# VIS4ROB-lab/HyperSLAM

Hardware: AMD Instinct MI355X
Metric: residual blocks linearised per second (LM iteration = linearise + Schur + solve + update), 128-control-point window (higher is better)
Workload: dtype f64

## Files before the change

hyperslam_amd/csrc/capi.hip:

```cpp
#include "host_tables.hpp"
#include "host_launch.hpp"
#include "tracker.hpp"

template <class Drop>
static int drop_rows(int n, Drop&& drop, std::vector<double>* stamp, std::vector<double>* meas, int width, std::vector<int32_t>* a = nullptr, std::vector<int32_t>* b = nullptr) {
  int w = 0;
  for (int i = 0; i < n; ++i) {
    if (drop(i)) continue;
    if (w != i) {
      (*stamp)[w] = (*stamp)[i];
      for (int c = 0; c < width; ++c) (*meas)[size_t(width) * w + c] = (*meas)[size_t(width) * i + c];
      if (a) (*a)[w] = (*a)[i];
      if (b) (*b)[w] = (*b)[i];
    }
    ++w;
  }
  stamp->resize(w), meas->resize(size_t(width) * w);
  if (a) a->resize(w);
  if (b) b->resize(w);
  return n - w;
}

extern "C" {

int hs_version(void) { return 1; }
const char* hs_arch(void) { return "gfx950"; }

int hs_create(int device, void* stream, hs_problem** out) {
  if (!out) return HS_ERR_INVALID;
  *out = nullptr;
  int count = 0;
  if (hipGetDeviceCount(&count) != hipSuccess || device < 0 || device >= count) return HS_ERR_DEVICE;
  hs_problem* p = new hs_problem();
  p->device = device;
  if (const char* e = std::getenv("HS_REFERENCE_LITERAL")) p->inertial_mode = std::atoi(e) ? HS_INERTIAL_AS_REFERENCE : HS_INERTIAL_EXACT;
  if (const char* e = std::getenv("HS_STAGE_TIMING")) p->stage_timing = std::atoi(e) != 0;
  if (const char* e = std::getenv("HS_HOST_TIMING")) p->host_timing = std::atoi(e) != 0;
  if (hipSetDevice(device) != hipSuccess) {
    delete p;
    return HS_ERR_DEVICE;
  }
  {
    int cus = 0;
    if (hipDeviceGetAttribute(&cus, hipDeviceAttributeMultiprocessorCount, device) == hipSuccess && cus > 0) p->n_cu = cus;
  }
  if (stream) {
    p->stream = static_cast<hipStream_t>(stream);
  } else {
    if (hipStreamCreateWithFlags(&p->stream, hipStreamNonBlocking) != hipSuccess) {
      delete p;
      return HS_ERR_DEVICE;
    }
    p->own_stream = true;
  }
  if (hipHostMalloc(reinterpret_cast<void**>(&p->h_state), sizeof(DevState), hipHostMallocDefault) != hipSuccess) {
    delete p;
    return HS_ERR_DEVICE;
  }
  warm_kernels(device);
  if (set_func_attributes(p) != HS_OK || ensure_side_stream(p) != HS_OK) {
    const std::string e = p->err;
    std::fprintf(stderr, "hyperslam_hip: %s\n", e.c_str());
    delete p;
    return HS_ERR_DEVICE;
  }
  *out = p;
  return HS_OK;
}

int hs_destroy(hs_problem* p) {
  if (!p) return HS_OK;
  if (p->host_timing && p->host_calls) {
    std::fprintf(stderr, "hs host timing over %d hs_solve calls [ms per call]: structure + tables %.4f, uploads %.4f, launches %.4f, wait %.4f\n", p->host_calls,
                 p->host_ms[0] / p->host_calls, p->host_ms[1] / p->host_calls, p->host_ms[2] / p->host_calls, p->host_ms[3] / p->host_calls);
    const size_t n = p->host_log.size() / 4, h = n / 2;
    double m[4] = {0, 0, 0, 0};
    for (size_t i = h; i < n; ++i)
      for (int c = 0; c < 4; ++c) m[c] += p->host_log[4 * i + c] / double(n - h);
    std::fprintf(stderr, "hs host timing, second half of the calls: structure + tables %.4f, uploads %.4f, launches %.4f, wait %.4f\n", m[0], m[1], m[2], m[3]);
    if (const char* e = std::getenv("HS_HOST_TIMING"); e && std::atoi(e) >= 2)
      for (size_t i = 0; i < n; ++i)
        std::fprintf(stderr, "hs host timing call %zu: structure + tables %.4f, uploads %.4f, launches %.4f, wait %.4f\n", i, p->host_log[4 * i],
                     p->host_log[4 * i + 1], p->host_log[4 * i + 2], p->host_log[4 * i + 3]);
  }
  if (p->scratch) hs_destroy(p->scratch), p->scratch = nullptr;
  (void)hipSetDevice(p->device);
  (void)hipStreamSynchronize(p->stream);
  for (hipEvent_t e : p->events) (void)hipEventDestroy(e);
  if (p->ev_fork) (void)hipEventDestroy(p->ev_fork);
  if (p->ev_join) (void)hipEventDestroy(p->ev_join);
  if (p->ev_irec) (void)hipEventDestroy(p->ev_irec);
  if (p->side) (void)hipStreamDestroy(p->side);
  if (p->h_state) (void)hipHostFree(p->h_state);
  if (p->h_result) (void)hipHostFree(p->h_result);
  if (p->rccl_comm && rccl_api()) (void)rccl_api()->CommDestroy(static_cast<ncclComm_t>(p->rccl_comm));
  if (p->own_stream) (void)hipStreamDestroy(p->stream);
  delete p;
  return HS_OK;
}

const char* hs_last_error(const hs_problem* p) { return p ? p->err.c_str() : "null handle"; }

static double knot_tolerance(double t0, double dt, int n_cp) {
  return std::max(1e-6 * dt, 8.0 * 2.220446049250313e-16 * std::max(std::fabs(t0), std::fabs(t0 + n_cp * dt)));
}

int hs_set_spline(hs_problem* p, int order, double t0, double dt, int n_cp, const double* cp, const uint8_t* cp_constant, int rc, int tc) {
  if (!p) return HS_ERR_INVALID;
  if (order < 2 || order > hsd::kMaxOrder) HS_FAIL(HS_ERR_INVALID, "spline order out of range");
  if (n_cp < order || !(dt > 0) || !cp) HS_FAIL(HS_ERR_INVALID, "need n_cp >= order, dt > 0 and a control-point table");
  const double knot_tol = knot_tolerance(t0, dt, n_cp);
  for (int j = 0; j < n_cp; ++j)
    if (!(std::fabs(cp[8 * j + 7] - (t0 + j * dt)) <= knot_tol))
      HS_FAIL(HS_ERR_KNOTS, "control-point stamps are not t0 + j dt (row " + std::to_string(j) + "): the spline basis is uniform, a table with a hole or non-uniform knots is refused");
  const bool same_structure = p->k == order && p->t0 == t0 && p->dt == dt && p->n_cp == n_cp && p->rot_const == (rc != 0) && p->trans_const == (tc != 0) &&
                              p->cp.size() == size_t(8) * n_cp;
  bool same_values = same_structure && std::memcmp(p->cp.data(), cp, sizeof(double) * 8 * n_cp) == 0;
  for (int j = 0; same_values && j < n_cp; ++j) same_values = p->cp_const[j] == (cp_constant ? cp_constant[j] : 0);
  if (same_values && !p->device_ahead) return HS_OK;
  p->k = order, p->t0 = t0, p->dt = dt, p->n_cp = n_cp;
  p->cp.assign(cp, cp + size_t(8) * n_cp);
  p->cp_const.assign(n_cp, 0);
  if (cp_constant) p->cp_const.assign(cp_constant, cp_constant + n_cp);
  p->rot_const = rc != 0, p->trans_const = tc != 0;
  p->touch(same_structure ? unsigned(hs_problem::vCp) : unsigned(hs_problem::kAll));
  return HS_OK;
}

static const char* kCameraShardMessage = "free camera blocks (hs_set_camera_constancy) are not supported on sharded handles (world > 1)";

int hs_set_cameras(hs_problem* p, int n, const double* T_bs, const double* intr, const double* dist) {
  if (!p) return HS_ERR_INVALID;
  if (n < 0 || n > 0xffff || (n && (!T_bs || !intr || !dist))) HS_FAIL(HS_ERR_INVALID, "bad camera table");
  const bool same_count = p->n_cam == n && p->cam.size() == size_t(kCamStride) * n;
  const std::vector<double> before = p->cam;
  p->n_cam = n;
  p->cam.assign(size_t(kCamStride) * n, 0.0);
  for (int i = 0; i < n; ++i) {
    double* c = &p->cam[size_t(kCamStride) * i];
    std::memcpy(c, T_bs + 7 * i, 56), std::memcpy(c + 7, intr + 4 * i, 32), std::memcpy(c + 11, dist + 4 * i, 32);
  }
  if (same_count && before == p->cam) return HS_OK;
  if (!same_count) p->cam_const.clear();
  p->touch(same_count ? unsigned(hs_problem::vCam) : unsigned(hs_problem::vCam | hs_problem::kVis));
  return HS_OK;
}

int hs_set_camera_constancy(hs_problem* p, int n, const uint8_t* constant) {
  if (!p) return HS_ERR_INVALID;
  std::vector<uint8_t> flags;
  if (constant) {
    if (n != p->n_cam) HS_FAIL(HS_ERR_INVALID, "hs_set_camera_constancy: n must equal the camera count of hs_set_cameras");
    flags.resize(size_t(3) * n);
    bool any_free = false;
    for (size_t i = 0; i < flags.size(); ++i) flags[i] = constant[i] ? 1 : 0, any_free |= !flags[i];
    if (!any_free) flags.clear();
  }
  if (flags == p->cam_const) return HS_OK;
  p->cam_const.swap(flags);
  p->touch(hs_problem::kTail);
  return HS_OK;
}

int hs_set_camera_estimation(hs_problem* p, int enabled) {
  if (!p) return HS_ERR_INVALID;
  const bool on = enabled != 0;
  if (on == p->cam_estimation) return HS_OK;
  p->cam_estimation = on;
  if (camera_columns(p, nullptr)) p->touch(hs_problem::kTail);
  return HS_OK;
}

int hs_get_cameras(hs_problem* p, double* T_bs, double* intr, double* dist) {
  if (!p) return HS_ERR_INVALID;
  for (int i = 0; i < p->n_cam; ++i) {
    const double* c = &p->cam[size_t(kCamStride) * i];
// ... 615 lines not shown
  }
  for (int d = 0; d < n_lm; ++d)
    if (lm_status[d])
      HS_FAIL(HS_ERR_NUMERIC, "hs_compute_covariance: rank deficient at landmark " + std::to_string(p->vs.table_of_dev[d]) +
                                  " (its observations do not fix all three coordinates)");
  p->cov_np = np, p->cov_ncb = ncb, p->cov_nb = nb, p->cov_nlm = n_lm;
  p->cov_valid = true;
  return HS_OK;
}

int hs_get_covariance(hs_problem* p, double* cp_blocks, double* cp_band, double* landmarks, double* border) {
  if (!p) return HS_ERR_INVALID;
  if (!p->cov_valid) HS_FAIL(HS_ERR_STATE, "hs_get_covariance: no covariance of the current state (call hs_compute_covariance after the last change)");
  const int np = p->cov_np, ncb = p->cov_ncb, nb = p->cov_nb, n_lm = p->cov_nlm, n_cp = np / 6, bw = ncb / 6;
  hipStream_t s = p->stream;
  std::vector<double> band, lm;
  if (cp_blocks || cp_band) {
    band.resize(size_t(np) * ncb);
    HIP_TRY(hipMemcpyAsync(band.data(), p->d_cov_band.p, band.size() * 8, hipMemcpyDeviceToHost, s));
  }
  if (landmarks && n_lm) {
    lm.resize(size_t(9) * n_lm);
    HIP_TRY(hipMemcpyAsync(lm.data(), p->d_cov_lm.p, lm.size() * 8, hipMemcpyDeviceToHost, s));
  }
  if (border && nb) HIP_TRY(hipMemcpyAsync(border, p->d_cov_bb.p, size_t(nb) * nb * 8, hipMemcpyDeviceToHost, s));
  HIP_TRY(hipStreamSynchronize(s));
  for (int i = 0; i < n_cp && (cp_blocks || cp_band); ++i)
    for (int j = 0; j < bw; ++j)
      for (int a = 0; a < 6; ++a)
        for (int b = 0; b < 6; ++b) {
          const double v = i + j < n_cp ? band[size_t(6 * i + a) * ncb + 6 * j + b] : 0.0;
          if (cp_band) cp_band[((size_t(i) * bw + j) * 6 + a) * 6 + b] = v;
          if (cp_blocks && j == 0) cp_blocks[(size_t(i) * 6 + a) * 6 + b] = v;
        }
  if (landmarks)
    for (int d = 0; d < n_lm; ++d) std::memcpy(landmarks + size_t(9) * p->vs.table_of_dev[d], lm.data() + size_t(9) * d, 9 * sizeof(double));
  return HS_OK;
}

int hs_sample_covariance(hs_problem* p, int n, const double* stamps, double* cov) {
  if (!p || n < 0 || (n && (!stamps || !cov))) return HS_ERR_INVALID;
  if (!p->cov_valid) HS_FAIL(HS_ERR_STATE, "hs_sample_covariance: no covariance of the current state (call hs_compute_covariance after the last change)");
  if (n == 0) return HS_OK;
  const int k = p->k, n_seg = p->n_cp - k + 1;
  for (int i = 0; i < n; ++i) {
    const int f = h_segment_first(stamps[i], p->t0, p->dt, k);
    if (f < 0 || f >= n_seg) HS_FAIL(HS_ERR_INVALID, "stamp outside the valid range of the spline");
  }
  hipStream_t s = p->stream;
  DBuf<double> d_st, d_out;
  std::vector<double> st(stamps, stamps + n);
  HIP_TRY(d_st.upload(st, s));
  HIP_TRY(d_out.reserve(size_t(36) * n));
  const int grid = (n + kBlock / 64 - 1) / (kBlock / 64);
  HS_ORDER_SWITCH(k, k_cov_sample<K><<<grid, kBlock, 0, s>>>(p->T, p->d_cov_band.p, n, d_st.p, d_out.p));
  HIP_TRY(hipGetLastError());
  HIP_TRY(hipMemcpyAsync(cov, d_out.p, size_t(36) * n * 8, hipMemcpyDeviceToHost, s));
  HIP_TRY(hipStreamSynchronize(s));
  return HS_OK;
}

int hs_set_weights(hs_problem* p, int type, const double* weights) {
  if (!p) return HS_ERR_INVALID;
  if (type < HS_PIXEL || type > HS_INERTIAL) HS_FAIL(HS_ERR_INVALID, "unknown factor type");
  const int nr = type == HS_PIXEL ? 2 : (type == HS_BEARING ? 1 : 6);
  if (weights)
    p->weights[type].assign(weights, weights + nr * nr);
  else
    p->weights[type].clear();
  return HS_OK;
}

int hs_set_guard(int enabled) {
  GuardRegistry::flag() = enabled != 0 ? 1 : 0;
  return HS_OK;
}

int hs_set_stage_timing(hs_problem* p, int enabled) {
  if (!p) return HS_ERR_INVALID;
  p->stage_timing = enabled != 0;
  return HS_OK;
}

int hs_solve(hs_problem* p, int max_iterations, hs_summary* summary, hs_iteration* iterations) {
  if (!p || !summary) return HS_ERR_INVALID;
  if (p->has_weights()) HS_FAIL(HS_ERR_INVALID, kWeightsMessage);
  if (max_iterations < 0 || max_iterations > kMaxIterations) HS_FAIL(HS_ERR_INVALID, "max_iterations out of range");
  if (camera_columns(p, nullptr)) {
    if (p->world > 1) HS_FAIL(HS_ERR_STATE, kCameraShardMessage);
    if (!p->cam_estimation)
      HS_FAIL(HS_ERR_STATE, "hs_solve: free camera blocks (hs_set_camera_constancy) are not supported by the solver in this version; "
                            "hs_reduced_system builds their system (DESIGN.md section 13)");
  }
  p->results_cached = false;
  p->cov_valid = false;
  int rc = prepare(p);
  if (rc) return rc;
  const bool spec = speculative_solve(p);
  const bool deferred = (fused_visual_only(p) || (spec && !commit_inline(p))) && !(p->T.debug_flags & 67108864);
  const bool fold = fold_decision_into_build(p, deferred);
  rc = reset_state(p, max_iterations, 1e4, spec ? (deferred ? 2 : 1) : (deferred ? 4 : 0));
  if (rc) return rc;
  hipStream_t s = p->stream;
  const auto host_t3 = std::chrono::steady_clock::now();
  const bool stages = p->stage_timing;
  const size_t n_ev = size_t(6) * max_iterations + 1;
  const size_t ev_cand = size_t(4) * max_iterations + 1;
  while (p->events.size() < n_ev) {
    hipEvent_t e;
    HIP_TRY(hipEventCreate(&e));
    p->events.push_back(e);
  }
  std::vector<hipEvent_t>& ev = p->events;
  HIP_TRY(hipEventRecord(ev[0], s));
  for (int it = 0; it < max_iterations; ++it) {
    if (it == 0 || !spec) {
      HS_ORDER_SWITCH(p->k, rc = launch_linearize<K>(p, true));
      if (rc) return rc;
    }
    if (stages && !p->fused) HIP_TRY(hipEventRecord(ev[4 * it + 1], s));
    hipEvent_t after_build = stages && p->fused ? ev[4 * it + 1] : nullptr;
    HS_ORDER_SWITCH(p->k, rc = launch_build<K>(p, after_build, it > 0, it > 0 && fold));
    if (rc) return rc;
    if (stages) HIP_TRY(hipEventRecord(ev[4 * it + 2], s));
    rc = launch_factor(p);
    if (rc) return rc;
    if (stages) HIP_TRY(hipEventRecord(ev[4 * it + 3], s));
    const bool lin_cand = spec && it + 1 < max_iterations;
    hipEvent_t* lin_ev = stages && lin_cand ? &ev[ev_cand + 2 * it] : nullptr;
    HS_ORDER_SWITCH(p->k, rc = launch_update<K>(p, lin_cand, deferred, lin_ev, fold && it + 1 < max_iterations));
    if (rc) return rc;
    if (deferred && it + 1 == max_iterations) launch_commit(p);
    if (stages || it + 1 == max_iterations) HIP_TRY(hipEventRecord(ev[4 * it + 4], s));
  }
  if (max_iterations == 0) {
    HS_ORDER_SWITCH(p->k, rc = launch_linearize<K>(p, false, true));
    if (rc) return rc;
    k_pack_exchange<<<1, kBlock, 0, s>>>(p->T, 0);
    rc = exchange(p, p->T.xbuf + p->T.xo_cost, 1);
    if (rc) return rc;
    k_cost_reduce<<<1, kBlock, 0, s>>>(p->T);
  }
  DevState& st = *p->h_state;
  const auto host_t4 = std::chrono::steady_clock::now();
  if (p->want_results) {
    const size_t n_cp8 = p->cp.size(), n_lm3 = p->lm.size(), n_b = p->has_imu ? p->bias_g.size() : 0, total = n_cp8 + n_lm3 + 2 * n_b + 3;
    if (total > p->h_result_cap) {
      if (p->h_result) (void)hipHostFree(p->h_result);
      p->h_result = nullptr, p->h_result_cap = 0;
      HIP_TRY(hipHostMalloc(reinterpret_cast<void**>(&p->h_result), 2 * total * sizeof(double), hipHostMallocDefault));
      p->h_result_cap = 2 * total;
    }
    double* h = p->h_result;
    HIP_TRY(hipMemcpyAsync(h, p->d_cp.p, n_cp8 * 8, hipMemcpyDeviceToHost, s));
    if (n_lm3) HIP_TRY(hipMemcpyAsync(h + n_cp8, p->d_lm.p, n_lm3 * 8, hipMemcpyDeviceToHost, s));
    if (n_b) {
      HIP_TRY(hipMemcpyAsync(h + n_cp8 + n_lm3, p->d_bias_g.p, n_b * 8, hipMemcpyDeviceToHost, s));
      HIP_TRY(hipMemcpyAsync(h + n_cp8 + n_lm3 + n_b, p->d_bias_a.p, n_b * 8, hipMemcpyDeviceToHost, s));
    }
    if (p->has_imu) HIP_TRY(hipMemcpyAsync(h + n_cp8 + n_lm3 + 2 * n_b, p->d_gravity.p, 24, hipMemcpyDeviceToHost, s));
  }
  if (p->T.nc && max_iterations > 0) HIP_TRY(hipMemcpyAsync(p->cam.data(), p->d_cam.p, p->cam.size() * 8, hipMemcpyDeviceToHost, s));
  HIP_TRY(hipMemcpyAsync(&st, p->d_state.p, sizeof(st), hipMemcpyDeviceToHost, s));
  HIP_TRY(hipStreamSynchronize(s));
  if (max_iterations > 0) p->device_ahead = true;
  p->results_cached = p->want_results;
  if (p->host_timing) {
    const auto host_t5 = std::chrono::steady_clock::now();
    const double tl = std::chrono::duration<double, std::milli>(host_t4 - host_t3).count(), tw = std::chrono::duration<double, std::milli>(host_t5 - host_t4).count();
    p->host_ms[2] += tl, p->host_ms[3] += tw;
    p->host_log.insert(p->host_log.end(), {p->host_prepare[0], p->host_prepare[1], tl, tw});
    p->host_prepare[0] = p->host_prepare[1] = 0;
    ++p->host_calls;
  }
  std::memset(summary, 0, sizeof(*summary));
  summary->initial_cost = st.records[0].cost;
  summary->final_cost = st.cost;
  summary->num_iterations = st.num_iterations;
  summary->num_successful_steps = st.num_successful;
  summary->termination = st.termination;
  summary->num_residual_blocks = p->T.n_vis + p->T.n_pri + p->T.n_ine;
  if (!stages) summary->linearize_ms = summary->schur_ms = summary->solve_ms = summary->update_ms = -1.0;
  for (int it = 0; stages && it < max_iterations; ++it) {
    float t[4] = {0, 0, 0, 0};
    for (int k = 0; k < 4; ++k) (void)hipEventElapsedTime(&t[k], ev[4 * it + k], ev[4 * it + k + 1]);
    summary->linearize_ms += t[0], summary->schur_ms += t[1], summary->solve_ms += t[2], summary->update_ms += t[3];
    if (spec && it + 1 < max_iterations) {
      float tc = 0;
      (void)hipEventElapsedTime(&tc, ev[ev_cand + 2 * it], ev[ev_cand + 2 * it + 1]);
      summary->linearize_ms += tc, summary->update_ms -= tc;
    }
  }
  if (max_iterations > 0) {
    float t = 0;
    (void)hipEventElapsedTime(&t, ev[0], ev[4 * max_iterations]);
    summary->total_ms = t;
  }
  if (iterations) {
    std::memset(iterations, 0, sizeof(hs_iteration) * (size_t(max_iterations) + 1));
    const int n = std::min(st.num_iterations, max_iterations);
    for (int i = 0; i <= n; ++i) iterations[i] = st.records[i];
  }
  if (st.chol_failed && st.termination == HS_FAILURE)
    p->err = st.chol_failed == 2 ? "two-ended solve: the partner workgroup did not arrive within 2 s" : "reduced system not positive definite";
  return guard_check(p);
}

#if HS_PROFILE_HOOKS
extern "C" int hs_debug_read(hs_problem* p, double* dst, int n) {
  if (!p || !dst) return HS_ERR_INVALID;
  HIP_TRY(hipMemcpyAsync(dst, p->d_xpart.p, size_t(n) * 8, hipMemcpyDeviceToHost, p->stream));
  HIP_TRY(hipStreamSynchronize(p->stream));
  return HS_OK;
}
#endif

int hs_snapshot(hs_problem* p) {
  if (!p) return HS_ERR_INVALID;
  int rc = prepare(p);
  if (rc) return rc;
  HIP_TRY(p->d_cp_snap.reserve(p->cp.size()));
  HIP_TRY(p->d_lm_snap.reserve(p->lm.size() + 1));
  HIP_TRY(hipMemcpyAsync(p->d_cp_snap.p, p->d_cp.p, p->cp.size() * 8, hipMemcpyDeviceToDevice, p->stream));
  if (p->n_lm) HIP_TRY(hipMemcpyAsync(p->d_lm_snap.p, p->d_lm.p, p->lm.size() * 8, hipMemcpyDeviceToDevice, p->stream));
  if (p->has_imu) {
    HIP_TRY(p->d_bias_g_snap.reserve(p->bias_g.size() + 1));
    HIP_TRY(p->d_bias_a_snap.reserve(p->bias_a.size() + 1));
    HIP_TRY(p->d_gravity_snap.reserve(3));
    HIP_TRY(hipMemcpyAsync(p->d_bias_g_snap.p, p->d_bias_g.p, p->bias_g.size() * 8, hipMemcpyDeviceToDevice, p->stream));
    HIP_TRY(hipMemcpyAsync(p->d_bias_a_snap.p, p->d_bias_a.p, p->bias_a.size() * 8, hipMemcpyDeviceToDevice, p->stream));
    HIP_TRY(hipMemcpyAsync(p->d_gravity_snap.p, p->d_gravity.p, 24, hipMemcpyDeviceToDevice, p->stream));
  }
  p->cam_snap = p->cam;
  p->has_snapshot = true;
  return HS_OK;
}

int hs_restore(hs_problem* p) {
  if (!p) return HS_ERR_INVALID;
  if (!p->has_snapshot || p->dirty) HS_FAIL(HS_ERR_STATE, "hs_restore without a valid hs_snapshot");
  p->results_cached = false;
  p->cov_valid = false;
  HIP_TRY(hipMemcpyAsync(p->d_cp.p, p->d_cp_snap.p, p->cp.size() * 8, hipMemcpyDeviceToDevice, p->stream));
  if (p->n_lm) HIP_TRY(hipMemcpyAsync(p->d_lm.p, p->d_lm_snap.p, p->lm.size() * 8, hipMemcpyDeviceToDevice, p->stream));
  if (p->has_imu) {
    HIP_TRY(hipMemcpyAsync(p->d_bias_g.p, p->d_bias_g_snap.p, p->bias_g.size() * 8, hipMemcpyDeviceToDevice, p->stream));
    HIP_TRY(hipMemcpyAsync(p->d_bias_a.p, p->d_bias_a_snap.p, p->bias_a.size() * 8, hipMemcpyDeviceToDevice, p->stream));
    HIP_TRY(hipMemcpyAsync(p->d_gravity.p, p->d_gravity_snap.p, 24, hipMemcpyDeviceToDevice, p->stream));
  }
  if (p->cam != p->cam_snap && p->cam.size() == p->cam_snap.size()) {
    p->cam = p->cam_snap;
    HIP_TRY(hipMemcpyAsync(p->d_cam.p, p->cam.data(), p->cam.size() * 8, hipMemcpyHostToDevice, p->stream));
    HIP_TRY(hipStreamSynchronize(p->stream));
  }
  return HS_OK;
}

int hs_rccl_unique_id(char id[128]) {
  static_assert(sizeof(ncclUniqueId) == 128, "ncclUniqueId is 128 bytes");
  if (!id) return HS_ERR_INVALID;
  RcclApi* api = rccl_api();
  if (!api) return HS_ERR_DEVICE;
  ncclUniqueId u;
  if (api->GetUniqueId(&u) != ncclSuccess) return HS_ERR_DEVICE;
  std::memcpy(id, &u, 128);
  return HS_OK;
}

int hs_rccl_init(hs_problem* p, const char id[128], int rank, int world) {
  if (!p || !id || world < 1 || rank < 0 || rank >= world) return HS_ERR_INVALID;
  RcclApi* api = rccl_api();
  if (!api) HS_FAIL(HS_ERR_DEVICE, "librccl.so could not be loaded");
  HIP_TRY(hipSetDevice(p->device));
  if (p->rccl_comm) {
    (void)api->CommDestroy(static_cast<ncclComm_t>(p->rccl_comm));
    p->rccl_comm = nullptr;
  }
  ncclUniqueId u;
  std::memcpy(&u, id, 128);
  ncclComm_t comm = nullptr;
  const ncclResult_t r = api->CommInitRank(&comm, world, u, rank);
  if (r != ncclSuccess) HS_FAIL(HS_ERR_DEVICE, std::string("ncclCommInitRank failed: ") + (api->GetErrorString ? api->GetErrorString(r) : "?"));
  p->rccl_comm = comm;
  return HS_OK;
}

int hs_rccl_shutdown(hs_problem* p) {
  if (!p) return HS_ERR_INVALID;
  if (p->rccl_comm && rccl_api()) {
    (void)hipStreamSynchronize(p->stream);
    (void)rccl_api()->CommDestroy(static_cast<ncclComm_t>(p->rccl_comm));
  }
  p->rccl_comm = nullptr;
  return HS_OK;
}

int hs_exchange_info(hs_problem* p, int32_t* rccl_ranks, int64_t* doubles_per_linearisation, int64_t* doubles_per_decision) {
  if (!p) return HS_ERR_INVALID;
  if (rccl_ranks) {
    int n = 0;
    if (p->rccl_comm && rccl_api() && rccl_api()->CommCount) {
      const ncclResult_t r = rccl_api()->CommCount(static_cast<ncclComm_t>(p->rccl_comm), &n);
      if (r != ncclSuccess) HS_FAIL(HS_ERR_DEVICE, "ncclCommCount failed");
    }
    *rccl_ranks = n;
  }
  if (doubles_per_linearisation) *doubles_per_linearisation = p->dirty ? 0 : p->T.x_count1;
  if (doubles_per_decision) *doubles_per_decision = 5;
  return HS_OK;
}

int hs_set_allreduce(hs_problem* p, hs_allreduce_fn fn, void* user) {
  if (!p) return HS_ERR_INVALID;
  p->allreduce = fn, p->allreduce_user = user;
  return HS_OK;
}

int hs_set_shard(hs_problem* p, int rank, int world, int min_band_blocks) {
  if (!p) return HS_ERR_INVALID;
  if (world < 1 || rank < 0 || rank >= world || min_band_blocks < 0) HS_FAIL(HS_ERR_INVALID, "bad shard description");
  p->rank = rank, p->world = world, p->min_bw = min_band_blocks;
  p->touch(hs_problem::kAll);
  return HS_OK;
}

int hs_band_blocks(hs_problem* p) {
  if (!p) return -1;
  if (prepare(p) != HS_OK) return -1;
  return p->T.bw;
}

// ... 601 lines not shown
```

hyperslam_amd/csrc/host_launch.hpp:

```cpp
#pragma once
#include "host_tables.hpp"

namespace {

int reset_state(hs_problem* p, int max_iterations, double radius, int spec = 0) {
  k_reset_state<<<1, 64, 0, p->stream>>>(p->d_state.p, max_iterations, radius, spec);
  HIP_TRY(hipGetLastError());
  return HS_OK;
}

size_t cp_lds_bytes(const hs_problem* p) { return size_t(8) * p->n_cp * sizeof(double); }
template <int K>
size_t lin_lds_bytes(const hs_problem* p) {
  return (cp_lds_bytes(p) <= 24 * 1024 ? cp_lds_bytes(p) : 0) + size_t(lin_block<K>()) * (8 + 12 * K + 2) * sizeof(double);
}

__global__ void k_noop() {}

static int ensure_side_stream(hs_problem* p) {
  if (!p->side) {
    HIP_TRY(hipStreamCreateWithFlags(&p->side, hipStreamNonBlocking));
    HIP_TRY(hipEventCreateWithFlags(&p->ev_fork, hipEventDisableTiming));
    HIP_TRY(hipEventCreateWithFlags(&p->ev_join, hipEventDisableTiming));
    HIP_TRY(hipEventCreateWithFlags(&p->ev_irec, hipEventDisableTiming));
// ... 15 lines not shown
    const int rc = ensure_side_stream(p);
    if (rc) return rc;
    HIP_TRY(hipEventRecord(p->ev_fork, s));
    HIP_TRY(hipStreamWaitEvent(p->side, p->ev_fork, 0));
  }
  if (T.n_vis && !p->fused) k_linearize_visual<K><<<p->nb_vis, lin_block<K>(), lin_lds_bytes<K>(p), s>>>(T, T.v_rec, T.v_pos, 1, T.cost_part, nullptr);
  if (T.n_vis && p->fused && visual_cost_only) k_cost_visual<K><<<p->nb_vis, kBlock, cp_lds_bytes(p), s>>>(T, T.cp, T.lm, T.cost_part);
  if (T.n_pri) k_linearize_prior<K><<<p->nb_pri, kBlock, cp_lds_bytes(p), s>>>(T, T.p_rec, T.cost_part + p->nb_vis, nullptr);
  if (T.n_ine)
    k_linearize_inertial<K, 4><<<p->nb_ine, kInertialBlock * K, cp_lds_bytes(p), p->side_imu ? p->side : s>>>(T, T.i_rec, 1, T.cost_part + p->nb_vis + p->nb_pri,
                                                                                                        nullptr);
  if (p->side_imu) HIP_TRY(hipEventRecord(p->ev_irec, p->side));
  HIP_TRY(hipGetLastError());
  return HS_OK;
}

struct RcclApi {
  void* lib = nullptr;
  ncclResult_t (*GetUniqueId)(ncclUniqueId*) = nullptr;
  ncclResult_t (*CommInitRank)(ncclComm_t*, int, ncclUniqueId, int) = nullptr;
  ncclResult_t (*AllReduce)(const void*, void*, size_t, ncclDataType_t, ncclRedOp_t, ncclComm_t, hipStream_t) = nullptr;
  ncclResult_t (*CommDestroy)(ncclComm_t) = nullptr;
  ncclResult_t (*CommCount)(const ncclComm_t, int*) = nullptr;
  const char* (*GetErrorString)(ncclResult_t) = nullptr;
};
static RcclApi* rccl_api() {
  static RcclApi api;
  static bool tried = false;
  if (!tried) {
    tried = true;
    for (const char* name : {"librccl.so.1", "librccl.so", "/opt/rocm/lib/librccl.so.1"}) {
      api.lib = dlopen(name, RTLD_NOW | RTLD_GLOBAL);
      if (api.lib) break;
    }
    if (api.lib) {
      api.GetUniqueId = reinterpret_cast<decltype(api.GetUniqueId)>(dlsym(api.lib, "ncclGetUniqueId"));
      api.CommInitRank = reinterpret_cast<decltype(api.CommInitRank)>(dlsym(api.lib, "ncclCommInitRank"));
      api.AllReduce = reinterpret_cast<decltype(api.AllReduce)>(dlsym(api.lib, "ncclAllReduce"));
      api.CommDestroy = reinterpret_cast<decltype(api.CommDestroy)>(dlsym(api.lib, "ncclCommDestroy"));
      api.GetErrorString = reinterpret_cast<decltype(api.GetErrorString)>(dlsym(api.lib, "ncclGetErrorString"));
      api.CommCount = reinterpret_cast<decltype(api.CommCount)>(dlsym(api.lib, "ncclCommCount"));
      if (!api.GetUniqueId || !api.CommInitRank || !api.AllReduce || !api.CommDestroy) api.lib = nullptr;
    }
  }
  return api.lib ? &api : nullptr;
}

int exchange(hs_problem* p, double* buf, int64_t count) {
  if (p->rccl_comm) {
    const ncclResult_t r = rccl_api()->AllReduce(buf, buf, size_t(count), ncclDouble, ncclSum, static_cast<ncclComm_t>(p->rccl_comm), p->stream);
    if (r != ncclSuccess) HS_FAIL(HS_ERR_DEVICE, std::string("ncclAllReduce failed: ") + (rccl_api()->GetErrorString ? rccl_api()->GetErrorString(r) : "?"));
    return HS_OK;
  }
  if (!p->allreduce) return HS_OK;
  if (p->allreduce(p->allreduce_user, buf, count, p->stream) != 0) HS_FAIL(HS_ERR_DEVICE, "all-reduce hook reported a failure");
  return HS_OK;
}

static int border_zero_wgs(const Tables& T) { return std::min(64, (T.nb * T.nb + T.nb + kPbThreads - 1) / kPbThreads); }

static bool factor_two_ended_la(const hs_problem* p) {
  const Tables& T = p->T;
  const int n_blk = T.np / 6;
  return T.nb == 0 && !(T.debug_flags & 4) && la_compute_waves(T.bw) > 0 && !HS_AB(T.debug_flags, 131072) && n_blk >= 4 * T.bw && T.Sb2 && !(T.debug_flags & 2048);
}

int mfma_window_tiles(int bw);
static bool factor_two_ended_any(const hs_problem* p) {
  const Tables& T = p->T;
  const int n_blk = T.np / 6;
  const bool la_ok = !(T.debug_flags & 4) && la_compute_waves(T.bw) > 0;
  const int nt = HS_AB(T.debug_flags, 131072) ? mfma_window_tiles(T.bw) : 0;
  if (T.nc) return false;
  return (la_ok || nt) && (T.nb == 0 || (!nt && !(T.debug_flags & 536870912) && (T.nb + kBorderCols - 1) / kBorderCols <= 512)) && n_blk >= 4 * T.bw && T.Sb2 &&
         !(T.debug_flags & 2048);
}
static bool use_dense_mx(const hs_problem* p, int* f0) {
  const Tables& T = p->T;
  const int n_blk = T.np / 6;
  *f0 = (T.debug_flags & 262144) ? 0 : std::min(p->frozen_prefix, n_blk - 1);
  return !factor_two_ended_any(p) && !HS_AB(T.debug_flags, 131072) && dense_mx_fits(n_blk - *f0, T.nb) && !(T.debug_flags & 8);
}

template <int K>
int launch_build(hs_problem* p, hipEvent_t after_build = nullptr, bool scaling_fixed = false, bool fold = false) {
  const Tables& T = p->T;
  hipStream_t s = p->stream;
  p->bookkeep = false;
  const bool fused = p->fused;
  const bool pair = !fused && T.n_lm > 0 && p->n_group_wg > 0 && p->n_group_wg + p->n_seg_wg <= 2048 && !(T.debug_flags & 1024);
  const bool side_imu = p->side_imu;
  const bool fork = !fused && T.n_lm > 0 && !pair && !side_imu;
  if (fused && fold) {
    Tables Tf = T;
    Tf.fold_decision = 1, Tf.fold_epoch = ++p->join_epoch;
    k_build_visual<K><<<p->nb_vis + 1, kBlock, p->build_lds, s>>>(Tf, p->build_R, p->build_L, 1);
  } else if (fused)
    k_build_visual<K><<<p->nb_vis, kBlock, p->build_lds, s>>>(T, p->build_R, p->build_L, 1);
  if (fused && T.wide_q) k_landmark_gram_wide<<<landmark_gram_wide_grid(T.sp.n_cp, T.bw), kGramWideThreads, 0, s>>>(T);
  if (fused && after_build) HIP_TRY(hipEventRecord(after_build, s));
  if (fork) {
    const int rc = ensure_side_stream(p);
    if (rc) return rc;
    HIP_TRY(hipEventRecord(p->ev_fork, s));
    HIP_TRY(hipStreamWaitEvent(p->side, p->ev_fork, 0));
  }
  hipStream_t sb = side_imu ? p->side : s;
  const bool gather_flag = side_imu && T.nb && !p->allreduce && !p->rccl_comm && p->world == 1 && !(T.debug_flags & 16384) &&
                           !(T.debug_flags & 8388608);
  const unsigned gather_epoch = gather_flag ? ++p->join_epoch : 0u;
  if (side_imu && T.nb) {
    k_border_pb<K><<<dim3(T.sp.n_cp + border_zero_wgs(T), p->n_split), kPbThreads, 0, sb>>>(T);
    Tables Tg = T;
    Tg.gather_epoch = gather_epoch;
    k_border_bb<K><<<T.n_bias, kBlock, 0, sb>>>(Tg);
    HIP_TRY(hipEventRecord(p->ev_join, p->side));
  }
  bool irec_ready = !side_imu;
  auto need_irec = [&]() -> hipError_t {
    if (irec_ready) return hipSuccess;
    irec_ready = true;
    return hipStreamWaitEvent(s, p->ev_irec, 0);
  };
  if (!pair && !(side_imu && T.n_lm) && p->n_seg_wg) {
    HIP_TRY(need_irec());
    k_seg_gram<K><<<p->n_seg_wg, kBlock, kSegStage * sizeof(double), fork ? p->side : s>>>(T);
  }
  if (fork) HIP_TRY(hipEventRecord(p->ev_join, p->side));
  if (T.n_lm && !fused) {
    const int grid = (T.n_lm + kBlock / 64 - 1) / (kBlock / 64);
    if (6 * T.bw <= 128)
      k_landmark<K, 2, 2><<<grid, kBlock, 0, s>>>(T);
    else if (T.debug_flags & 4194304)
      k_landmark<K, 4, 1><<<grid, kBlock, 0, s>>>(T);
    else
      k_landmark_rows<K, 4><<<T.n_lm, kBlock, 0, s>>>(T);
  }
  if (T.n_lm && p->n_group_wg && !fused) {
    const int ntile = T.bw * (T.bw + 1) / 2;
    const int batch = std::max(2, std::min(kGroupBatch, int(48 * 1024 / (size_t(18) * T.bw * sizeof(double)))));
    const size_t lds = std::max((size_t(batch) * 18 * T.bw + 4 * batch) * sizeof(double), size_t(128) * 42 * sizeof(double));
    const dim3 grid(p->n_group_wg);
    if (pair) {
      HIP_TRY(need_irec());
      const size_t lds2 = std::max(lds, kSegStage * sizeof(double));
      const dim3 grid2(p->n_group_wg + p->n_seg_wg);
      if (ntile <= kBlock)
        k_gram_pair<K, 1><<<grid2, kBlock, lds2, s>>>(T, batch, p->n_group_wg);
      else if (ntile <= 2 * kBlock)
        k_gram_pair<K, 2><<<grid2, kBlock, lds2, s>>>(T, batch, p->n_group_wg);
      else
        k_gram_pair<K, 4><<<grid2, kBlock, lds2, s>>>(T, batch, p->n_group_wg);
    } else if (ntile <= kBlock)
      k_group_gram<1><<<grid, kBlock, lds, s>>>(T, batch);
    else if (ntile <= 2 * kBlock)
      k_group_gram<2><<<grid, kBlock, lds, s>>>(T, batch);
    else
      k_group_gram<4><<<grid, kBlock, lds, s>>>(T, batch);
  }
  if (side_imu && T.n_lm && !pair && p->n_seg_wg) {
    HIP_TRY(need_irec());
    k_seg_gram<K><<<p->n_seg_wg, kBlock, kSegStage * sizeof(double), s>>>(T);
  }
  if (fork) HIP_TRY(hipStreamWaitEvent(s, p->ev_join, 0));
  Tables Ta = T;
  const bool dense_mx = use_dense_mx(p, &Ta.dense_f0);
  const bool direct = scaling_fixed && fused && !T.nb && !p->allreduce && !p->rccl_comm && p->world == 1 && (factor_two_ended_la(p) || dense_mx) &&
                      !(T.debug_flags & 4096);
  if (direct && dense_mx) Ta.dense = p->d_dense_ut.p + size_t(kDenseLd) * kDenseLd;
  if (fused && T.bw * (T.bw + 1) / 2 > kBlock)
    k_assemble_wide<K><<<dim3(T.sp.n_cp, 6), kAsmWideThreads, 0, s>>>(Ta, direct ? 1 : 0);
  else
    k_assemble<K><<<dim3(T.sp.n_cp, 6), kAsmThreads, 0, s>>>(Ta, direct ? 1 : 0);
  if (direct) {
    p->bookkeep = true;
    HIP_TRY(hipGetLastError());
    return HS_OK;
  }
// ... 280 lines not shown
static bool speculative_solve(const hs_problem* p) {
  const Tables& T = p->T;
  return !p->fused && T.n_vis > 0 && !T.n_pri && !T.n_ine && !T.nb && !(T.debug_flags & 1073741824);
}
static bool fused_visual_only(const hs_problem* p) {
  const Tables& T = p->T;
  return p->fused && !T.n_pri && !T.n_ine && !T.nb;
}

static bool fold_decision_into_build(const hs_problem* p, bool deferred_commit) {
  return fused_visual_only(p) && deferred_commit && !p->allreduce && !p->rccl_comm && p->world == 1 && !(p->T.debug_flags & 32768);
}

static bool commit_inline(const hs_problem* p) {
  const Tables& T = p->T;
  return !p->allreduce && !p->rccl_comm && 8 * T.sp.n_cp + 3 * T.n_lm + 8 * T.n_bias <= kCommitInline && !(T.debug_flags & 16777216);
}

template <int K>
int launch_update(hs_problem* p, bool linearize_candidate = false, bool deferred_commit = false, hipEvent_t* lin_events = nullptr, bool fold_next = false) {
  const Tables& T = p->T;
  hipStream_t s = p->stream;
  const bool local_decision = !p->allreduce && !p->rccl_comm;
  const bool inline_commit = commit_inline(p) && !deferred_commit;
  const bool cps_here = p->fused && deferred_commit;
  const int decide_here = inline_commit ? 2 : local_decision ? (cps_here ? 3 : 1) : 0;
  const bool merged = p->fused && local_decision && !(T.debug_flags & 134217728);
  Tables calib_tables[2];
  if (T.nc) {
    k_calib_candidate<<<1, kBlock, 0, s>>>(T, p->d_cam_cand.p, T.n_norm_part);
    calib_tables[0] = calib_tables[1] = T;
    calib_tables[0].cam = p->d_cam_cand.p, calib_tables[1].n_norm_part = T.n_norm_part + 1;
  }
  const Tables &Tc = T.nc ? calib_tables[0] : T, &Td = T.nc ? calib_tables[1] : T;
  if (p->fused) {
    const int nb_pri = merged && T.n_pri ? p->nb_pri : 0, nb_ine = merged && T.n_ine ? p->nb_ine : 0;
    const size_t lds = std::max(size_t(update_lds_doubles(T.bw, p->build_R, p->build_L)), size_t(8 * T.sp.n_cp + 8 * T.n_bias + 4)) * 8;
    if (T.nc)
      k_update_visual<K, true><<<p->nb_vis + T.n_norm_part + nb_pri + nb_ine, kBlock, lds, s>>>(Tc, p->build_R, p->build_L, p->nb_vis, nb_pri, nb_ine);
    else
      k_update_visual<K><<<p->nb_vis + T.n_norm_part + nb_pri + nb_ine, kBlock, lds, s>>>(T, p->build_R, p->build_L, p->nb_vis, nb_pri, nb_ine);
    if (T.n_pri && !merged) k_cost_prior<K><<<p->nb_pri, kBlock, cp_lds_bytes(p), s>>>(T, T.cp_cand, T.cand_part + p->nb_vis);
    if (T.n_ine && !merged)
      k_cost_inertial<K, 4><<<p->nb_ine, kInertialBlock, cp_lds_bytes(p), s>>>(T, T.cp_cand, T.bias_g_cand, T.bias_a_cand, T.gravity_cand,
                                                                          T.cand_part + p->nb_vis + p->nb_pri);
  } else if (T.nc)
    k_backsub_retract<true><<<T.n_lm_part + T.n_norm_part, kBlock, 0, s>>>(T);
  else
    k_backsub_retract<false><<<T.n_lm_part + T.n_norm_part, kBlock, 0, s>>>(T);
  if (p->fused) {
  } else if (linearize_candidate) {
    if (lin_events) HIP_TRY(hipEventRecord(lin_events[0], s));
    k_linearize_visual<K><<<p->nb_vis, lin_block<K>(), lin_lds_bytes<K>(p), s>>>(T, nullptr, T.v_pos, 1, T.cand_part, nullptr, T.cp_cand, T.lm_cand);
    if (lin_events) HIP_TRY(hipEventRecord(lin_events[1], s));
  } else if ((T.n_ine || T.n_pri) && !(T.debug_flags & 33554432)) {
    k_cost_all<K, 4><<<p->nb_vis + p->nb_pri + p->nb_ine, kBlock, cp_lds_bytes(p), s>>>(Tc, T.cp_cand, T.lm_cand, T.bias_g_cand, T.bias_a_cand, T.gravity_cand,
                                                                                       T.cand_part, p->nb_vis, p->nb_pri);
  } else {
    if (T.n_vis) k_cost_visual<K><<<p->nb_vis, kBlock, cp_lds_bytes(p), s>>>(Tc, T.cp_cand, T.lm_cand, T.cand_part);
    if (T.n_pri) k_cost_prior<K><<<p->nb_pri, kBlock, cp_lds_bytes(p), s>>>(T, T.cp_cand, T.cand_part + p->nb_vis);
    if (T.n_ine)
      k_cost_inertial<K, 4><<<p->nb_ine, kInertialBlock, cp_lds_bytes(p), s>>>(T, T.cp_cand, T.bias_g_cand, T.bias_a_cand, T.gravity_cand,
                                                                          T.cand_part + p->nb_vis + p->nb_pri);
  }
  if (fold_next) return HS_OK;
  k_pack_decision<<<1, kBlock, 0, s>>>(Td, decide_here);
  HIP_TRY(hipGetLastError());
  const int rc = exchange(p, T.xbuf + T.xo_dec, 5);
  if (rc) return rc;
  if (!local_decision) k_decide<<<1, kBlock, 0, s>>>(T, cps_here ? 1 : 0);
  const int nb_commit = std::max((std::max(8 * T.sp.n_cp, 3 * T.n_lm) + kBlock - 1) / kBlock, 1);
  if (!inline_commit && !deferred_commit) k_commit<<<nb_commit, kBlock, 0, s>>>(T);
  if (T.nc) k_calib_commit<<<1, kBlock, 0, s>>>(T, p->d_cam.p, p->d_cam_cand.p);
  HIP_TRY(hipGetLastError());
  return HS_OK;
}

static void launch_commit(hs_problem* p) {
  const Tables& T = p->T;
  const int nb_commit = std::max((std::max(8 * T.sp.n_cp, 3 * T.n_lm) + kBlock - 1) / kBlock, 1);
  k_commit<<<nb_commit, kBlock, 0, p->stream>>>(T);
}

template <int K>
static void warm_kernels_of_order() {
  hipFuncAttributes fa;
  const void* kernels[] = {
      reinterpret_cast<const void*>(&k_build_visual<K>), reinterpret_cast<const void*>(&k_update_visual<K>), reinterpret_cast<const void*>(&k_linearize_visual<K>), reinterpret_cast<const void*>(&k_linearize_prior<K>),
      reinterpret_cast<const void*>(&k_linearize_inertial<K, 4>), reinterpret_cast<const void*>(&k_landmark<K, 2, 2>),
      reinterpret_cast<const void*>(&k_landmark<K, 4, 1>), reinterpret_cast<const void*>(&k_landmark_rows<K, 4>),
      reinterpret_cast<const void*>(&k_gram_pair<K, 1>), reinterpret_cast<const void*>(&k_gram_pair<K, 2>), reinterpret_cast<const void*>(&k_gram_pair<K, 4>),
      reinterpret_cast<const void*>(&k_seg_gram<K>), reinterpret_cast<const void*>(&k_assemble<K>), reinterpret_cast<const void*>(&k_assemble_wide<K>), reinterpret_cast<const void*>(&k_border_pb<K>),
      reinterpret_cast<const void*>(&k_border_bb<K>), reinterpret_cast<const void*>(&k_cost_visual<K>), reinterpret_cast<const void*>(&k_cost_prior<K>),
      reinterpret_cast<const void*>(&k_cost_inertial<K, 4>), reinterpret_cast<const void*>(&k_cost_all<K, 4>),
      reinterpret_cast<const void*>(&k_process_tracks<K>), reinterpret_cast<const void*>(&k_sample_trajectory<K>)};
  for (const void* k : kernels) (void)hipFuncGetAttributes(&fa, k);
}
static void warm_kernels(int device) {
  static std::mutex mu;
  static std::vector<int> done;
  std::lock_guard<std::mutex> lock(mu);
  if (std::find(done.begin(), done.end(), device) != done.end()) return;
  done.push_back(device);
  hipFuncAttributes fa;
  const void* kernels[] = {
      reinterpret_cast<const void*>(&k_group_gram<1>), reinterpret_cast<const void*>(&k_group_gram<2>), reinterpret_cast<const void*>(&k_group_gram<4>),
      reinterpret_cast<const void*>(&k_pack_exchange), reinterpret_cast<const void*>(&k_cost_reduce), reinterpret_cast<const void*>(&k_finalize_reduced),
      reinterpret_cast<const void*>(&k_finalize_border), reinterpret_cast<const void*>(&k_reduce_partials), reinterpret_cast<const void*>(&k_factor_decoupled_rows),
      reinterpret_cast<const void*>(&k_dense_factor), reinterpret_cast<const void*>(&k_dense_solve_mx), reinterpret_cast<const void*>(&k_band_factor_wide), reinterpret_cast<const void*>(&k_band_factor<1>),
      reinterpret_cast<const void*>(&k_band_factor<2>), reinterpret_cast<const void*>(&k_band_factor_la<1, 3>), reinterpret_cast<const void*>(&k_band_factor_la<1, 4>),
      reinterpret_cast<const void*>(&k_band_backward), reinterpret_cast<const void*>(&k_band_backward_sb), reinterpret_cast<const void*>(&k_border_forward),
      reinterpret_cast<const void*>(&k_border_forward2),
      reinterpret_cast<const void*>(&k_border_schur), reinterpret_cast<const void*>(&k_border_solve), reinterpret_cast<const void*>(&k_border_solve_reg<3>), reinterpret_cast<const void*>(&k_border_solve_reg<4>),
      reinterpret_cast<const void*>(&k_border_solve_reg<5>), reinterpret_cast<const void*>(&k_border_solve_reg<6>), reinterpret_cast<const void*>(&k_border_solve_reg<7>),
      reinterpret_cast<const void*>(&k_border_solve_reg<8>), reinterpret_cast<const void*>(&k_border_apply), reinterpret_cast<const void*>(&k_backsub_retract<false>),
      reinterpret_cast<const void*>(&k_pack_decision), reinterpret_cast<const void*>(&k_decide), reinterpret_cast<const void*>(&k_commit),
      reinterpret_cast<const void*>(&k_reset_state), reinterpret_cast<const void*>(&k_scatter_uploads)};
  for (const void* k : kernels) (void)hipFuncGetAttributes(&fa, k);
  warm_kernels_of_order<4>();
  warm_kernels_of_order<5>();
  warm_kernels_of_order<6>();
}

int set_func_attributes(hs_problem* p) {
  hipFuncAttributes fa;
  HIP_TRY(hipFuncGetAttributes(&fa, reinterpret_cast<const void*>(&k_band_factor<2>)));
  p->chol_lds_max = 160 * 1024 - int(fa.sharedSizeBytes);
  HIP_TRY(hipFuncSetAttribute(reinterpret_cast<const void*>(&k_band_factor<1>), hipFuncAttributeMaxDynamicSharedMemorySize, p->chol_lds_max));
  HIP_TRY(hipFuncSetAttribute(reinterpret_cast<const void*>(&k_band_factor<2>), hipFuncAttributeMaxDynamicSharedMemorySize, p->chol_lds_max));
  HIP_TRY(hipFuncSetAttribute(reinterpret_cast<const void*>(&k_band_factor_la<1, 3>), hipFuncAttributeMaxDynamicSharedMemorySize, p->chol_lds_max));
  HIP_TRY(hipFuncSetAttribute(reinterpret_cast<const void*>(&k_band_factor_la<1, 4>), hipFuncAttributeMaxDynamicSharedMemorySize, p->chol_lds_max));
  for (int k = 4; k <= 6; ++k) HS_ORDER_SWITCH(k, {
    HIP_TRY(hipFuncSetAttribute(reinterpret_cast<const void*>(&k_seg_gram<K>), hipFuncAttributeMaxDynamicSharedMemorySize, 64 * 1024));
    HIP_TRY(hipFuncSetAttribute(reinterpret_cast<const void*>(&k_gram_pair<K, 1>), hipFuncAttributeMaxDynamicSharedMemorySize, 64 * 1024));
    HIP_TRY(hipFuncSetAttribute(reinterpret_cast<const void*>(&k_gram_pair<K, 2>), hipFuncAttributeMaxDynamicSharedMemorySize, 64 * 1024));
    HIP_TRY(hipFuncSetAttribute(reinterpret_cast<const void*>(&k_gram_pair<K, 4>), hipFuncAttributeMaxDynamicSharedMemorySize, 64 * 1024));
    HIP_TRY(hipFuncSetAttribute(reinterpret_cast<const void*>(&k_build_visual<K>), hipFuncAttributeMaxDynamicSharedMemorySize, 158 * 1024));
    HIP_TRY(hipFuncSetAttribute(reinterpret_cast<const void*>(&k_update_visual<K>), hipFuncAttributeMaxDynamicSharedMemorySize, 158 * 1024));
    HIP_TRY(hipFuncSetAttribute(reinterpret_cast<const void*>(&k_update_visual<K, true>), hipFuncAttributeMaxDynamicSharedMemorySize, 158 * 1024));
    HIP_TRY(hipFuncSetAttribute(reinterpret_cast<const void*>(&k_linearize_visual<K>), hipFuncAttributeMaxDynamicSharedMemorySize, 150 * 1024));
  });
  HIP_TRY(hipFuncSetAttribute(reinterpret_cast<const void*>(&k_dense_solve_mx), hipFuncAttributeMaxDynamicSharedMemorySize, int(kDxLdsDoubles * sizeof(double))));
  HIP_TRY(hipFuncSetAttribute(reinterpret_cast<const void*>(&k_border_solve_reg<5>), hipFuncAttributeMaxDynamicSharedMemorySize, 160 * 1024 - 1024));
  HIP_TRY(hipFuncSetAttribute(reinterpret_cast<const void*>(&k_border_solve_reg<6>), hipFuncAttributeMaxDynamicSharedMemorySize, 160 * 1024 - 1024));
  HIP_TRY(hipFuncSetAttribute(reinterpret_cast<const void*>(&k_border_solve_reg<7>), hipFuncAttributeMaxDynamicSharedMemorySize, 160 * 1024 - 1024));
  HIP_TRY(hipFuncSetAttribute(reinterpret_cast<const void*>(&k_border_solve_reg<8>), hipFuncAttributeMaxDynamicSharedMemorySize, 160 * 1024 - 1024));
  HIP_TRY(hipFuncSetAttribute(reinterpret_cast<const void*>(&k_border_forward), hipFuncAttributeMaxDynamicSharedMemorySize, 150 * 1024));
  HIP_TRY(hipFuncSetAttribute(reinterpret_cast<const void*>(&k_border_forward2), hipFuncAttributeMaxDynamicSharedMemorySize, 150 * 1024));
#if HS_PROFILE_HOOKS
  HIP_TRY(hipFuncSetAttribute(reinterpret_cast<const void*>(&k_band_backward2), hipFuncAttributeMaxDynamicSharedMemorySize, 150 * 1024));
#endif
  HIP_TRY(hipFuncSetAttribute(reinterpret_cast<const void*>(&k_band_backward_sb), hipFuncAttributeMaxDynamicSharedMemorySize, 150 * 1024));
  HIP_TRY(hipFuncSetAttribute(reinterpret_cast<const void*>(&k_band_backward), hipFuncAttributeMaxDynamicSharedMemorySize, 150 * 1024));
  HIP_TRY(hipFuncSetAttribute(reinterpret_cast<const void*>(&k_border_solve), hipFuncAttributeMaxDynamicSharedMemorySize, 150 * 1024));
  return HS_OK;
}

}
```

hyperslam_amd/csrc/host_structure.hpp:

```cpp
#pragma once
#include <algorithm>
#include <cmath>
#include <cstdint>
#include <numeric>
#include <string>
#include <vector>

#include "../../include/hyperslam_hip.h"
#include "device_math.hpp"

namespace hs {

inline double h_binom(int n, int r) {
  if (r < 0 || r > n) return 0.0;
  double v = 1.0;
  for (int i = 1; i <= r; ++i) v = v * (n - r + i) / i;
  return v;
}

inline hsd::BasisCoef make_basis_coef(int k) {
  hsd::BasisCoef b;
  for (double& v : b.c) v = 0.0;
  std::vector<double> M(size_t(k) * k, 0.0);
  double fact = 1.0;
// ... 107 lines not shown
    std::vector<int>& start = vs->scratch_start;
    start.assign(in.n_cp + 2, 0);
    for (int t = 0; t < in.n_lm; ++t) start[std::min(cf[t], in.n_cp) + 1]++;
    for (int c = 0; c <= in.n_cp; ++c) start[c + 1] += start[c];
    vs->table_of_dev.resize(in.n_lm), vs->dev_of_table.resize(in.n_lm);
    for (int t = 0; t < in.n_lm; ++t) {
      const int d = start[std::min(cf[t], in.n_cp)]++;
      vs->table_of_dev[d] = t, vs->dev_of_table[t] = d;
    }
  }
  vs->lm_cfirst.resize(in.n_lm), vs->lm_ncp.resize(in.n_lm), vs->lm_yoff.resize(in.n_lm + 1), vs->lm_ptr.resize(in.n_lm + 1);
  vs->lm_yoff[0] = 0, vs->lm_ptr[0] = 0;
  vs->bw = in.k;
  for (int d = 0; d < in.n_lm; ++d) {
    const int t = vs->table_of_dev[d];
    if (cl[t] >= 0) {
      vs->lm_cfirst[d] = cf[t];
      vs->lm_ncp[d] = cl[t] - cf[t] + 1;
      vs->bw = std::max(vs->bw, vs->lm_ncp[d]);
    } else {
      vs->lm_cfirst[d] = in.n_cp;
      vs->lm_ncp[d] = 0;
    }
    vs->lm_yoff[d + 1] = vs->lm_yoff[d] + 18 * vs->lm_ncp[d];
    vs->lm_ptr[d + 1] = vs->lm_ptr[d] + cnt[t];
    cnt[t] = vs->lm_ptr[d];
  }
  vs->y_total = vs->lm_yoff[in.n_lm];
  vs->cf_ptr.assign(in.n_cp + 2, 0);
  for (int c = 0, d = 0; c <= in.n_cp + 1; ++c) {
    while (d < in.n_lm && vs->lm_cfirst[d] < c) ++d;
    vs->cf_ptr[c] = d;
  }
  vs->table_type.resize(n), vs->table_idx.resize(n), vs->lm_dev.resize(n), vs->first.resize(n), vs->pos.resize(n);
  auto pass_b = [&](const int32_t* lm, int count, int offset, int type) {
    for (int j = 0; j < count; ++j) {
      const int t = lm[j], q = cnt[t]++;
      vs->table_type[q] = type, vs->table_idx[q] = j, vs->lm_dev[q] = vs->dev_of_table[t], vs->first[q] = first[offset + j];
    }
  };
  pass_b(in.px_lm, in.n_px, 0, HS_PIXEL), pass_b(in.br_lm, in.n_br, in.n_px, HS_BEARING);
  {
    std::vector<int>& cur = vs->scratch_start;
    cur.assign(vs->seg_ptr.begin(), vs->seg_ptr.end() - 1);
    for (int q = 0; q < n; ++q) vs->pos[q] = cur[vs->first[q]]++;
  }
  return true;
}

inline bool build_chunks(const VisualStructure& vs, int n_cp, int R, int L, std::vector<int>* ch_ptr, std::vector<int>* gw_ptr, std::vector<int>* gw_cf,
                         std::vector<int>* ch_desc = nullptr) {
  int n_obs = int(vs.lm_ptr.size()) - 1;
  while (n_obs > 0 && vs.lm_ptr[n_obs] == vs.lm_ptr[n_obs - 1]) --n_obs;
  ch_ptr->clear(), gw_cf->clear();
  gw_ptr->assign(n_cp + 1, 0);
  for (int c = 0; c < n_cp; ++c) {
    const int d0 = std::min(vs.cf_ptr[c], n_obs), d1 = std::min(vs.cf_ptr[c + 1], n_obs);
    (*gw_ptr)[c] = int(gw_cf->size());
    if (d1 <= d0) continue;
    int d = d0;
    while (d < d1) {
      if (vs.lm_ptr[d + 1] - vs.lm_ptr[d] > R) return false;
      ch_ptr->push_back(d), gw_cf->push_back(c);
      int cnt = 0, e = d;
      while (e < d1 && e - d < L && cnt + (vs.lm_ptr[e + 1] - vs.lm_ptr[e]) <= R) cnt += vs.lm_ptr[e + 1] - vs.lm_ptr[e], ++e;
      d = e;
    }
  }
  (*gw_ptr)[n_cp] = int(gw_cf->size());
  ch_ptr->push_back(n_obs);
  gw_cf->push_back(0);
  if (ch_desc) {
    const int n = int(ch_ptr->size()) - 1;
    ch_desc->assign(size_t(8) * std::max(n, 1), 0);
    for (int w = 0; w < n; ++w) {
      const int lo = (*ch_ptr)[w], hi = (*ch_ptr)[w + 1];
      int* d = ch_desc->data() + 8 * w;
      d[0] = lo, d[1] = hi - lo, d[2] = vs.lm_cfirst[lo], d[3] = vs.lm_ptr[lo], d[4] = vs.lm_ptr[hi] - vs.lm_ptr[lo], d[5] = w;
    }
  }
  return true;
}

inline void order_chunks_for_dispatch(const VisualStructure& vs, int k, int n_cu, std::vector<int>* ch_desc, int n) {
  if (n <= 1 || n_cu <= 0) return;
  std::vector<int> weight(n), order(n);
  std::vector<int> cnt;
  for (int c = 0; c < n; ++c) {
    const int* d = ch_desc->data() + 8 * c;
    cnt.assign(size_t(vs.bw) + k + 1, 0);
    for (int q = d[3]; q < d[3] + d[4]; ++q) {
      const int o = vs.first[q] - d[2];
      if (o >= 0 && o < vs.bw) cnt[o]++;
    }
    int run = 0, best = 0;
    for (int o = 0; o < vs.bw + k; ++o) {
      run += (o < vs.bw ? cnt[o] : 0) - (o >= k ? cnt[o - k] : 0);
      best = std::max(best, run);
    }
    weight[c] = best, order[c] = c;
  }
  std::stable_sort(order.begin(), order.end(), [&](int a, int b) { return weight[a] > weight[b]; });
  std::vector<int> slot_chunk(n, -1);
  if (n > n_cu && n <= 2 * n_cu) {
    const int n_lone = 2 * n_cu - n, n_pair = n - n_cu;
    for (int i = 0; i < n_lone; ++i) slot_chunk[n_pair + i] = order[i];
    for (int i = 0; i < n_pair; ++i) slot_chunk[i] = order[n_lone + i], slot_chunk[n_cu + i] = order[n - 1 - i];
  } else {
    for (int i = 0; i < n; ++i) slot_chunk[i] = order[i];
  }
  std::vector<int> out(ch_desc->size(), 0);
  for (int w = 0; w < n; ++w) std::copy(ch_desc->begin() + 8 * slot_chunk[w], ch_desc->begin() + 8 * slot_chunk[w] + 8, out.begin() + 8 * w);
  ch_desc->swap(out);
}

template <class LdsBytes>
inline bool choose_build_geometry(int k, int R0, int L0, size_t lds_two, size_t lds_one, LdsBytes lds_bytes, int* R, int* L) {
  for (const size_t cap : {lds_two, lds_one}) {
    int r = R0, l = L0;
    while (lds_bytes(r, l) > cap && l > 4) --l;
    while (lds_bytes(r, l) > cap && r > 64) r -= 32;
    if (lds_bytes(r, l) <= cap) {
      *R = r, *L = l;
      return true;
    }
  }
  (void)k;
  return false;
}

}
```

hyperslam_amd/csrc/host_tables.hpp:

```cpp
#pragma once
#include <dlfcn.h>
#include <hip/hip_runtime.h>
#include <rccl/rccl.h>

#include <cstdio>
#include <cstdlib>
#include <chrono>
#include <cstring>
#include <string>
#include <mutex>
#include <vector>

#include "host_structure.hpp"
#include "kernels.hpp"

using namespace hs;

namespace {

struct UploadBatch {
  struct Seg {
    unsigned long long dst, off, bytes;
  };
  std::vector<Seg> segs;
// ... 176 lines not shown
  void touch(unsigned what) { changed |= what, dirty = true, cov_valid = false; }
  bool device_ahead = false;

  int k = 0, n_cp = 0;
  double t0 = 0, dt = 0;
  std::vector<double> cp;
  std::vector<uint8_t> cp_const;
  int rot_const = 0, trans_const = 0;
  int n_cam = 0;
  std::vector<double> cam;
  std::vector<uint8_t> cam_const;
  bool cam_estimation = false;
  std::vector<double> cam_snap;
  int n_sensor = 0;
  std::vector<double> sensor;
  int n_lm = 0;
  std::vector<double> lm;
  std::vector<uint8_t> lm_const;
  std::vector<double> px_stamp, px_meas, br_stamp, br_meas, pr_stamp, pr_meas, in_stamp, in_meas;
  std::vector<int32_t> px_lm, px_cam, br_lm, br_cam, pr_sensor;
  bool has_imu = false;
  double imu_T_bs[7], imu_i_g[6], imu_i_a[6], imu_S_g[9], imu_X_a[9];
  int kb = 4, n_bias = 0;
  double bias_t0 = 0, bias_dt = 1;
  std::vector<double> bias_g, bias_a;
  int bias_const = 0;
  double gravity[3] = {0, 0, -9.80665};
  int gravity_const = 1;
  int inertial_mode = HS_INERTIAL_AS_REFERENCE;
  hs_problem* scratch = nullptr;
  int frozen_prefix = 0;
  bool stage_timing = false;
  std::vector<double> weights[4];
  bool has_weights() const { return !weights[0].empty() || !weights[1].empty() || !weights[2].empty() || !weights[3].empty(); }
  UploadBatch batch;
  bool host_timing = false;
  double host_ms[5] = {0, 0, 0, 0, 0};
  int host_calls = 0;
  std::vector<double> host_log;
  double host_prepare[2] = {0, 0};
  double* h_result = nullptr;
  size_t h_result_cap = 0;
  bool want_results = false, results_cached = false;
  size_t vb_len = 0;
  int zeroed_np = -1, zeroed_ncb = -1;
  const void* zeroed_ptr[5] = {nullptr, nullptr, nullptr, nullptr, nullptr};

  VisualStructure vs;
  std::vector<int> pr_order;
  std::vector<int> pr_first, pr_seg_ptr;

  DBuf<double> d_cp, d_cp_cand, d_cam, d_sensor, d_lm, d_lm_cand;
  DBuf<uint8_t> d_cp_const, d_lm_const;
  DBuf<int> d_lm_ptr, d_lm_cfirst, d_lm_ncp, d_lm_yoff, d_cf_ptr;
  DBuf<double> d_lm_scale, d_lm_L, d_lm_yhat, d_lm_sb, d_lm_D2, d_lm_part, d_lm_gmax, d_gabs, d_Y;
  DBuf<double> d_v_stamp, d_v_meas, d_v_rec, d_v_rec_alt;
  DBuf<int> d_v_lm, d_v_info, d_v_first, d_v_pos, d_v_seg_ptr, d_v_dbgpos;
  DBuf<double> d_p_stamp, d_p_meas, d_p_rec;
  DBuf<double> d_i_stamp, d_i_meas, d_i_rec, d_bias_g, d_bias_a, d_bias_g_cand, d_bias_a_cand, d_gravity, d_gravity_cand;
  DBuf<int> d_i_first, d_i_first_bias, d_i_seg_ptr;
  DBuf<ImuParams> d_imu;
  std::vector<int> in_order, in_first, in_first_bias, in_seg_ptr, in_bias_ptr;
  int nb_ine = 0;
  DBuf<int> d_p_sensor, d_p_first, d_p_seg_ptr;
  DBuf<double> d_scale_p, d_Sb, d_Ub, d_Ubk, d_g_s, d_g_full, d_D2p, d_step_p, d_delta_p;
  DBuf<double> d_cost_part, d_cand_part, d_norm_part, d_dbg, d_dbg_cost;
  DBuf<DevState> d_state;
  DBuf<double> d_xbuf, d_xpart, d_segP, d_grpQ, d_Qw, d_Yt, d_gravity_part;
  int yt_stride = 0;
  bool wide_q = false;
  DBuf<double> d_Vb, d_Vb2, d_yt, d_yt2;
  DBuf<double> d_Sb2, d_g2, d_Ub2, d_Ubk2, d_ybuf2, d_win, d_xsol;
  DBuf<unsigned> d_join;
  DBuf<double> d_dense_ut;
  DBuf<double> d_bf_handover;
  unsigned join_epoch = 0;
  DBuf<int> d_gw_ptr, d_gw_cf, d_sw_ptr, d_sw_seg;
  int n_seg_wg = 0, n_group_wg = 0;
  bool fused = false;
  int dense_border_nb = -1;
  bool bookkeep = false;
  int build_R = 0, build_L = 0;
  size_t build_lds = 0;
  DBuf<int> d_ch_ptr, d_ch_desc;
  DBuf<double> d_ch_gmax;
  std::vector<int> h_ch_ptr, h_gw_ptr, h_gw_cf, h_ch_desc;
  DBuf<double> d_ybuf, d_scale_b, d_Spb, d_Sbb, d_gb_s, d_D2b, d_Zb, d_Cb, d_hb, d_xb, d_delta_b, d_bias_g_snap, d_bias_a_snap, d_gravity_snap;
  DBuf<int> d_i_bias_ptr, d_bfwd_start;
  int n_split = 1;
  int rank = 0, world = 1, min_bw = 0;
  DBuf<double> d_cp_snap, d_lm_snap;
  bool has_snapshot = false;
  DevState* h_state = nullptr;
  bool cov_valid = false;
  int cov_np = 0, cov_ncb = 0, cov_nb = 0, cov_nlm = 0;
  DBuf<double> d_cov_U, d_cov_sig, d_cov_Z, d_cov_X, d_cov_C, d_cov_Li, d_cov_band, d_cov_pb, d_cov_bb, d_cov_lm;
  DBuf<uint8_t> d_cov_const;
  DBuf<int> d_cov_status, d_cov_lm_status;
  int nc = 0;
  std::vector<int> calib_map;
  DBuf<int> d_calib_map;
  DBuf<double> d_calib_rec, d_calib_Yc, d_calib_part, d_cam_cand;
  DBuf<int> d_calib_bfwd;
  std::vector<hipEvent_t> events;
  hipStream_t side = nullptr;
  hipEvent_t ev_fork = nullptr, ev_join = nullptr, ev_irec = nullptr;
  bool side_imu = false;
  Tables T;
  int nb_vis = 0, nb_pri = 0, nb_cp = 0;
  int chol_lds_max = 64 * 1024;
  hs_allreduce_fn allreduce = nullptr;
  void* allreduce_user = nullptr;
  void* rccl_comm = nullptr;
};

static const char* kWeightsMessage =
    "a weight matrix is set (hs_set_weights): weights are applied by hs_linearize / hs_cost_function_evaluate; the solver runs the "
    "reference's production configuration, weights = nullptr (optimizer.cpp:191,214,236,255)";

#define HS_AB(flags, bit) (HS_PROFILE_HOOKS && ((flags) & (bit)))

#define HS_ORDER_SWITCH(k, ...)    \
  do {                             \
    if ((k) == 4) {                \
      constexpr int K = 4;         \
      __VA_ARGS__;                 \
    } else if ((k) == 5) {         \
      constexpr int K = 5;         \
      __VA_ARGS__;                 \
    } else {                       \
      constexpr int K = 6;         \
      __VA_ARGS__;                 \
    }                              \
  } while (0)

#define HS_FAIL(code, msg) \
  do {                     \
    p->err = (msg);        \
    return (code);         \
  } while (0)
#define HIP_TRY(expr)                                                                             \
  do {                                                                                            \
    const hipError_t e__ = (expr);                                                                \
    if (e__ != hipSuccess) {                                                                      \
      p->err = std::string(#expr) + ": " + hipGetErrorString(e__);                                \
      return HS_ERR_DEVICE;                                                                       \
    }                                                                                             \
  } while (0)

namespace {

int mfma_window_tiles(int bw);

static int camera_columns(const hs_problem* p, std::vector<int>* map) {
  if (map) map->clear();
  if (p->cam_const.empty()) return 0;
  std::vector<uint8_t> used(p->n_cam, 0);
  for (int32_t c : p->px_cam)
    if (c >= 0 && c < p->n_cam) used[c] = 1;
  for (int32_t c : p->br_cam)
    if (c >= 0 && c < p->n_cam) used[c] = 1;
  static const int first[3] = {0, 6, 10}, size[3] = {6, 4, 4};
  int n = 0;
  for (int c = 0; c < p->n_cam; ++c)
    for (int b = 0; b < 3; ++b)
      if (used[c] && !p->cam_const[3 * c + b])
        for (int j = 0; j < size[b]; ++j, ++n)
          if (map) map->push_back(c << 8 | (first[b] + j));
  return n;
}

static int upload_values(hs_problem* p, unsigned what) {
  hipStream_t s = p->stream;
  if (what & hs_problem::vCp) {
    HIP_TRY(p->d_cp.upload(p->cp, s));
    HIP_TRY(p->d_cp_cand.reserve(p->cp.size()));
// ... 295 lines not shown
                                  " control points, at most " + std::to_string(150 * 1024 / (6 * 8 * 8)) + " (6 n_cp x 8 doubles within 150 KiB)");
    if (nbd + 1 > 128 && (size_t(nbd + 1) * (nbd + 1) + nbd) * sizeof(double) > size_t(150) * 1024)
      HS_FAIL(HS_ERR_INVALID, "too many border unknowns for the LDS-resident dense solve of the border system: " + std::to_string(nbi) +
                                  " bias / gravity + " + std::to_string(p->nc) + " free camera coordinates = " + std::to_string(nbd) +
                                  ", at most 137 (hs_set_camera_estimation)");
  }
  if (nbi && size_t(np) * 8 * 8 > 150 * 1024) HS_FAIL(HS_ERR_INVALID, "window too long for the LDS-resident border forward sweep");
  if (nbi + 1 > 128 && (size_t(nbi + 1) * (nbi + 1) + nbi) * sizeof(double) > size_t(150) * 1024)
    HS_FAIL(HS_ERR_INVALID, "too many border unknowns (bias control points) for the LDS-resident dense solve of the border system: at most 22 bias control points per window");
  const int x_count0 = np * (ncb + 3) + np * nbd + nbd * nbd + nbd + 1 + p->world;
  const int x_count1 = x_count0 + 2 * p->nc;
  if (p->nc) {
    HIP_TRY(p->d_calib_map.upload(p->calib_map, s));
    HIP_TRY(p->d_calib_rec.reserve(size_t(std::max(n_vis, 1)) * (40 + 12 * k)));
    HIP_TRY(p->d_calib_Yc.reserve(size_t(std::max(p->n_lm, 1)) * 3 * p->nc));
    const int n_parts = (n_vis + kCalibRowChunk - 1) / kCalibRowChunk + (p->n_lm + kCalibLmChunk - 1) / kCalibLmChunk;
    HIP_TRY(p->d_calib_part.reserve(size_t(std::max(n_parts, 1)) * (p->nc * p->nc + 2 * p->nc)));
    HIP_TRY(p->d_cam_cand.reserve(size_t(kCamStride) * std::max(p->n_cam, 1)));
    HIP_TRY(p->d_calib_bfwd.upload(std::vector<int>((nbd + kBorderCols - 1) / kBorderCols + kSchurTile, 0), s));
  }
  HIP_TRY(p->d_ybuf.reserve(np));
  HIP_TRY(p->d_scale_b.reserve(nbd + 1));
  HIP_TRY(p->d_Spb.reserve(size_t(np) * nbd + 1));
  HIP_TRY(p->d_Sbb.reserve(size_t(nbd) * nbd + 1));
  HIP_TRY(p->d_gb_s.reserve(nbd + 1));
  HIP_TRY(p->d_D2b.reserve(nbd + 1));
  HIP_TRY(p->d_Zb.reserve(size_t(np) * nbd + 1));
  HIP_TRY(p->d_Cb.reserve(size_t(nbd) * nbd + 1));
  HIP_TRY(p->d_hb.reserve(nbd + 1));
  HIP_TRY(p->d_xb.reserve(nbd + 1));
  HIP_TRY(p->d_delta_b.reserve(nbd + 1));
  HIP_TRY(p->d_xbuf.reserve(size_t(x_count1) + 8));
  HIP_TRY(p->d_gravity_part.reserve(size_t(5) * std::max(p->n_bias, 1)));
  {
    const size_t nv = size_t(np) * ncb, pad = 64, vb_len = std::max(nv, size_t(576) * ((size_t(p->n_cp) + 3) / 4 + 1));
    p->vb_len = vb_len;
    HIP_TRY(p->d_Sb2.reserve(nv));
    for (DBuf<double>* b : {&p->d_Vb, &p->d_Vb2}) HIP_TRY(b->reserve(vb_len + pad));
    for (DBuf<double>* b : {&p->d_yt, &p->d_yt2}) HIP_TRY(b->reserve(size_t(np) + pad));
    const void* now[5] = {p->d_Sb2.p, p->d_Vb.p, p->d_Vb2.p, p->d_yt.p, p->d_yt2.p};
    if (p->zeroed_np != np || p->zeroed_ncb != ncb || std::memcmp(now, p->zeroed_ptr, sizeof(now)) != 0) {
      HIP_TRY(hipMemsetAsync(p->d_Sb2.p, 0, p->d_Sb2.cap * sizeof(double), s));
      for (DBuf<double>* b : {&p->d_Vb, &p->d_Vb2}) HIP_TRY(hipMemsetAsync(b->p + vb_len, 0, pad * sizeof(double), s));
      for (DBuf<double>* b : {&p->d_yt, &p->d_yt2}) HIP_TRY(hipMemsetAsync(b->p + np, 0, pad * sizeof(double), s));
      p->zeroed_np = np, p->zeroed_ncb = ncb, std::memcpy(p->zeroed_ptr, now, sizeof(now));
    }
  }
  HIP_TRY(p->d_g2.reserve(np));
  HIP_TRY(p->d_Ub2.reserve(size_t(np) * ncb));
  HIP_TRY(p->d_Ubk2.reserve(size_t(p->n_cp) * 24));
  HIP_TRY(p->d_ybuf2.reserve(np));
  HIP_TRY(p->d_xsol.reserve(np));
  HIP_TRY(p->d_win.reserve(size_t(6) * vs.bw * (ncb + 1)));
  HIP_TRY(p->d_dense_ut.reserve(size_t(2) * kDenseLd * kDenseLd));
  if (!p->d_join.p) {
    HIP_TRY(p->d_join.reserve(kGatherFlag + kProgressStride));
    HIP_TRY(hipMemsetAsync(p->d_join.p, 0, (kGatherFlag + kProgressStride) * sizeof(unsigned), s));
    p->join_epoch = 0;
  }
  p->n_split = std::max(1, std::min(16, 2048 / std::max(p->n_cp, 1)));
  HIP_TRY(p->d_xpart.reserve(size_t(x_count1) * p->n_split));
  {
    const int n_seg_ = p->n_cp - k + 1, nca = 6 * k, ntile = vs.bw * (vs.bw + 1) / 2;
    std::vector<int> sw_ptr(n_seg_ + 1, 0), sw_seg;
    for (int f = 0; f < n_seg_; ++f) {
      const int load = (p->fused ? 0 : vs.seg_ptr[f + 1] - vs.seg_ptr[f]) + 3 * (p->pr_seg_ptr[f + 1] - p->pr_seg_ptr[f]) +
                       (p->in_seg_ptr.empty() ? 0 : 3 * (p->in_seg_ptr[f + 1] - p->in_seg_ptr[f]));
      const int nw = p->fused ? (load + 95) / 96 : std::max(1, (load + 95) / 96);
      sw_ptr[f + 1] = sw_ptr[f] + nw;
      for (int w = 0; w < nw; ++w) sw_seg.push_back(f);
    }
    p->n_seg_wg = sw_ptr[n_seg_];
    sw_seg.push_back(0);
    HIP_TRY(p->d_sw_ptr.upload(sw_ptr, s));
    HIP_TRY(p->d_sw_seg.upload(sw_seg, s));
    const int per_wg = 12;
    std::vector<int> gw_ptr(p->n_cp + 1, 0), gw_cf;
    if (!(what & hs_problem::kVis)) {
    } else if (p->fused) {
      HIP_TRY(p->d_gw_ptr.upload(p->h_gw_ptr, s));
      HIP_TRY(p->d_gw_cf.upload(p->h_gw_cf, s));
      HIP_TRY(p->d_ch_ptr.upload(p->h_ch_ptr, s));
      HIP_TRY(p->d_ch_desc.upload(p->h_ch_desc, s));
      p->n_group_wg = int(p->h_ch_ptr.size()) - 1;
    } else {
      for (int c = 0; c < p->n_cp; ++c) {
        const int cnt = vs.cf_ptr[c + 1] - vs.cf_ptr[c], nw = (cnt + per_wg - 1) / per_wg;
        gw_ptr[c + 1] = gw_ptr[c] + nw;
        for (int w = 0; w < nw; ++w) gw_cf.push_back(c);
      }
      p->n_group_wg = gw_ptr[p->n_cp];
      gw_cf.push_back(0);
      HIP_TRY(p->d_gw_ptr.upload(gw_ptr, s));
      HIP_TRY(p->d_gw_cf.upload(gw_cf, s));
    }
    HIP_TRY(p->d_segP.reserve(size_t(p->n_seg_wg) * (size_t(nca) * nca + nca) + 1));
    HIP_TRY(p->d_grpQ.reserve(size_t(p->n_group_wg) * (size_t(ntile) * 36 + (p->fused ? 3 : 1) * 6 * vs.bw) + 1));
    {
      const char* env = std::getenv("HS_WIDE_Q");
      p->wide_q = p->fused && ntile > kBlock && !(env && std::atoi(env) == 0);
      if (p->wide_q) {
        HIP_TRY(p->d_Qw.reserve(size_t(6) * p->n_cp * (6 * vs.bw + 1) + 1));
        p->yt_stride = (p->n_lm + 63) / 64 * 64;
        HIP_TRY(p->d_Yt.reserve(size_t(18) * p->n_cp * p->yt_stride + 2));
      }
    }
  }
  HIP_TRY(p->d_state.reserve(1));

  Tables& T = p->T;
  std::memset(&T, 0, sizeof(T));
  p->dense_border_nb = -1;
  T.sp = Spline{k, p->n_cp, p->t0, p->dt, 1.0 / p->dt, p->rot_const, p->trans_const};
  T.basis = make_basis_coef(k);
  T.cp = p->d_cp.p, T.cp_cand = p->d_cp_cand.p, T.cp_const = p->d_cp_const.p;
  T.cam = p->d_cam.p, T.n_cam = p->n_cam, T.sensor = p->d_sensor.p;
  T.n_lm = p->n_lm, T.lm = p->d_lm.p, T.lm_cand = p->d_lm_cand.p, T.lm_const = p->d_lm_const.p;
  T.lm_ptr = p->d_lm_ptr.p, T.lm_cfirst = p->d_lm_cfirst.p, T.lm_ncp = p->d_lm_ncp.p, T.lm_yoff = p->d_lm_yoff.p, T.cf_ptr = p->d_cf_ptr.p;
  T.lm_scale = p->d_lm_scale.p, T.lm_L = p->d_lm_L.p, T.lm_yhat = p->d_lm_yhat.p, T.lm_sb = p->d_lm_sb.p, T.lm_D2 = p->d_lm_D2.p;
  T.lm_part = p->d_lm_part.p, T.n_lm_part = p->fused ? p->nb_vis : (p->n_lm + kBlock / 64 - 1) / (kBlock / 64), T.lm_gmax = p->d_lm_gmax.p, T.Y = p->d_Y.p;
  {
    int n_obs = p->n_lm;
    while (n_obs > 0 && vs.lm_ptr[n_obs] == vs.lm_ptr[n_obs - 1]) --n_obs;
    T.n_obs_lm = n_obs;
  }
  T.n_vis = n_vis, T.v_stamp = p->d_v_stamp.p, T.v_meas = p->d_v_meas.p, T.v_lm = p->d_v_lm.p, T.v_info = p->d_v_info.p;
  T.v_first = p->d_v_first.p, T.v_pos = p->d_v_pos.p, T.v_rec = p->d_v_rec.p, T.v_rec_alt = p->d_v_rec_alt.p, T.v_seg_ptr = p->d_v_seg_ptr.p;
  T.n_pri = n_pri, T.p_stamp = p->d_p_stamp.p, T.p_meas = p->d_p_meas.p, T.p_sensor = p->d_p_sensor.p, T.p_first = p->d_p_first.p;
  T.p_rec = p->d_p_rec.p, T.p_seg_ptr = p->d_p_seg_ptr.p;
  T.n_ine = n_ine, T.i_stamp = p->d_i_stamp.p, T.i_meas = p->d_i_meas.p, T.i_first = p->d_i_first.p, T.i_first_bias = p->d_i_first_bias.p;
  T.i_rec = p->d_i_rec.p, T.i_seg_ptr = p->d_i_seg_ptr.p, T.imu = p->d_imu.p;
  T.bias_basis = make_basis_coef(p->kb), T.kb = p->kb, T.n_bias = p->has_imu ? p->n_bias : 0, T.bias_t0 = p->bias_t0, T.bias_dt = p->bias_dt;
  T.bias_g = p->d_bias_g.p, T.bias_a = p->d_bias_a.p, T.bias_g_cand = p->d_bias_g_cand.p, T.bias_a_cand = p->d_bias_a_cand.p;
  T.gravity = p->d_gravity.p, T.gravity_cand = p->d_gravity_cand.p, T.bias_const = p->bias_const, T.gravity_const = p->gravity_const;
  T.inertial_literal = p->inertial_mode == HS_INERTIAL_AS_REFERENCE;
  T.nb = (p->has_imu ? 6 * p->n_bias + 2 : 0) + p->nc;
  T.nc = p->nc, T.calib_map = p->d_calib_map.p, T.calib_rec = p->d_calib_rec.p, T.calib_Yc = p->d_calib_Yc.p, T.calib_part = p->d_calib_part.p;
  T.n_seg = n_seg, T.bw = vs.bw, T.np = np;
  T.scale_p = p->d_scale_p.p, T.Sb = p->d_Sb.p, T.Ub = p->d_Ub.p, T.Ubk = p->d_Ubk.p, T.g_s = p->d_g_s.p, T.g_full = p->d_g_full.p, T.D2p = p->d_D2p.p, T.gabs = p->d_gabs.p;
  T.step_p = p->d_step_p.p, T.delta_p = p->d_delta_p.p;
  T.cost_part = p->d_cost_part.p, T.cand_part = p->d_cand_part.p, T.n_cost_part = p->nb_vis + p->nb_pri + p->nb_ine;
  if (size_t(T.n_cost_part) > p->d_cost_part.cap || size_t(T.n_cost_part) > p->d_cand_part.cap)
    HS_FAIL(HS_ERR_DEVICE, "internal: cost partial tables shorter than the grids that write them");
  T.norm_part = p->d_norm_part.p, T.n_norm_part = nb_norm;
  T.xbuf = p->d_xbuf.p;
  T.xpart = p->d_xpart.p, T.gravity_part = p->d_gravity_part.p, T.segP = p->d_segP.p, T.grpQ = p->d_grpQ.p, T.Qw = p->d_Qw.p, T.wide_q = p->wide_q && n_vis > 0 ? 1 : 0, T.Yt = p->d_Yt.p, T.yt_stride = p->yt_stride, T.gw_ptr = p->d_gw_ptr.p, T.gw_cf = p->d_gw_cf.p, T.sw_ptr = p->d_sw_ptr.p, T.sw_seg = p->d_sw_seg.p;
  T.xo_g = np * ncb, T.xo_gs = T.xo_g + np, T.xo_dj = T.xo_gs + np, T.xo_pb = T.xo_dj + np, T.xo_bb = T.xo_pb + np * nbd;
  T.xo_gb = T.xo_bb + nbd * nbd, T.xo_cost = T.xo_gb + nbd, T.xo_gmax = T.xo_cost + 1;
  T.ybuf = p->d_ybuf.p, T.ybuf2 = nullptr, T.y_split = np;
  T.fj[0] = FactorJob{T.Sb, T.g_s, T.Ub, T.Ubk, T.ybuf, nullptr, np / 6, -1};
  T.fj[1] = FactorJob{nullptr, nullptr, nullptr, nullptr, nullptr, nullptr, 0, -1};
  T.xsol = p->d_xsol.p, T.join_flag = p->d_join.p, T.join_epoch = 0;
  T.debug_flags = std::getenv("HS_DEBUG_FLAGS") ? std::atoi(std::getenv("HS_DEBUG_FLAGS")) : 0;
  {
    const bool la_ok = la_compute_waves(vs.bw) > 0, two_ended = la_ok && np / 6 >= 4 * vs.bw;
    const bool need = two_ended || (HS_AB(T.debug_flags, 131072) && mfma_window_tiles(vs.bw) > 0);
    T.Sb2 = need ? p->d_Sb2.p : nullptr, T.g2 = need ? p->d_g2.p : nullptr;
  }
  T.scale_b = p->d_scale_b.p, T.Spb = p->d_Spb.p, T.Sbb = p->d_Sbb.p, T.gb_s = p->d_gb_s.p, T.D2b = p->d_D2b.p;
  T.Zb = p->d_Zb.p, T.Cb = p->d_Cb.p, T.hb = p->d_hb.p, T.xb = p->d_xb.p, T.delta_b = p->d_delta_b.p, T.i_bias_ptr = p->d_i_bias_ptr.p, T.bfwd_start = p->nc ? p->d_calib_bfwd.p : p->d_bfwd_start.p;
  T.x_count1 = x_count1, T.xo_dec = x_count1, T.xo_cdj = x_count0;
  T.fused = p->fused ? 1 : 0, T.n_chunk = p->fused ? p->n_group_wg : 0, T.ch_ptr = p->d_ch_ptr.p, T.ch_desc = p->d_ch_desc.p;
  T.build_stream_lg = p->fused ? build_streams_packed(vs.bw, k) : 0;
  T.ch_gmax = p->d_ch_gmax.p;
  T.rank = p->rank, T.world = p->world;
  T.st = p->d_state.p;
  HIP_TRY(p->batch.flush(s));
  p->dirty = false, p->changed = 0;
  if ((what & hs_problem::kValues) == hs_problem::kValues) p->device_ahead = false;
  if (p->host_timing) {
    const auto host_t2 = std::chrono::steady_clock::now();
    p->host_prepare[0] = std::chrono::duration<double, std::milli>(host_t1 - host_t0).count();
    p->host_prepare[1] = std::chrono::duration<double, std::milli>(host_t2 - host_t1).count();
    p->host_ms[0] += p->host_prepare[0], p->host_ms[1] += p->host_prepare[1];
  }
  return HS_OK;
}


}
```

hyperslam_amd/csrc/kernels_aux.hpp:

```cpp
#pragma once
#include "kernels_common.hpp"

namespace hs {

template <int K>
__global__ void __launch_bounds__(kBlock) k_sample_trajectory(Tables T, int n, const double* stamps, double* pose, double* vel, double* acc) {
  HS_DYNAMIC_LDS(smem);
  double* cps = smem;
  stage_cps(T.cp, cps, 8 * T.sp.n_cp);
  const int i = blockIdx.x * blockDim.x + threadIdx.x;
  if (i >= n) return;
  double u;
  const int first = segment_of(stamps[i], T.sp.t0, T.sp.dt, K, &u);
  double lam[K], dlam[K], ddlam[K];
  basis_weights<K>(T.basis, u, T.sp.inv_dt, lam, dlam, ddlam, 2);
  SplineFull<K> S;
  spline_full<K, false>(cps + 8 * first, lam, dlam, ddlam, &S);
  double* o = pose + 7 * i;
  o[0] = S.q.x, o[1] = S.q.y, o[2] = S.q.z, o[3] = S.q.w, o[4] = S.p.x, o[5] = S.p.y, o[6] = S.p.z;
  if (vel) vel[6 * i] = S.w.x, vel[6 * i + 1] = S.w.y, vel[6 * i + 2] = S.w.z, vel[6 * i + 3] = S.v.x, vel[6 * i + 4] = S.v.y, vel[6 * i + 5] = S.v.z;
  if (acc) acc[6 * i] = S.al.x, acc[6 * i + 1] = S.al.y, acc[6 * i + 2] = S.al.z, acc[6 * i + 3] = S.a.x, acc[6 * i + 4] = S.a.y, acc[6 * i + 5] = S.a.z;
}

HSD V3 pixel_to_bearing(const double* cam, double u, double v) {
  const double xd = (u - cam[7]) / cam[9], yd = (v - cam[8]) / cam[10];
  const double k1 = cam[11], k2 = cam[12], p1 = cam[13], p2 = cam[14];
  double x = xd, y = yd;
  for (int it = 0; it < 20; ++it) {
    const double r2 = x * x + y * y, rad = 1 + k1 * r2 + k2 * r2 * r2;
    const double dx = 2 * p1 * x * y + p2 * (r2 + 2 * x * x), dy = p1 * (r2 + 2 * y * y) + 2 * p2 * x * y;
    x = (xd - dx) / rad, y = (yd - dy) / rad;
  }
  const double n = sqrt(x * x + y * y + 1);
  return V3{x / n, y / n, 1 / n};
}

template <int K>
__global__ void __launch_bounds__(kBlock) k_process_tracks(Tables T, double stamp, int n, const double* px0, const double* px1, double* b0o, double* b1o,
                                                           double* pwo) {
  HS_DYNAMIC_LDS(smem);
  double* cps = smem;
  stage_cps(T.cp, cps, 8 * T.sp.n_cp);
  const int i = blockIdx.x * blockDim.x + threadIdx.x;
  if (i >= n) return;
  const double* c0 = T.cam, *c1 = T.cam + 16;
  const V3 b0 = pixel_to_bearing(c0, px0[2 * i], px0[2 * i + 1]), b1 = pixel_to_bearing(c1, px1[2 * i], px1[2 * i + 1]);
  if (b0o) b0o[3 * i] = b0.x, b0o[3 * i + 1] = b0.y, b0o[3 * i + 2] = b0.z;
  if (b1o) b1o[3 * i] = b1.x, b1o[3 * i + 1] = b1.y, b1o[3 * i + 2] = b1.z;
  if (!pwo) return;
  double u;
  const int first = segment_of(stamp, T.sp.t0, T.sp.dt, K, &u);
  double lam[K], dlam[K], ddlam[K];
  basis_weights<K>(T.basis, u, T.sp.inv_dt, lam, dlam, ddlam, 0);
  Quat q_wb;
  V3 p_wb;
  spline_pose<K>(cps + 8 * first, lam, &q_wb, &p_wb);
  const Quat q_b0 = load_quat(c0), q_b1 = load_quat(c1);
  const V3 t_b0 = V3{c0[4], c0[5], c0[6]}, t_b1 = V3{c1[4], c1[5], c1[6]};
  const M3 R_wb = qmat(q_wb), R_b0 = qmat(q_b0), R_b1 = qmat(q_b1);
  const M3 R_01 = mul_tn(R_b0, R_b1);
  const V3 o = mul_t(R_b0, t_b1 - t_b0);
  const V3 d1 = mul(R_01, b1);
  const double a = dot(b0, b0), b = dot(b0, d1), c = dot(d1, d1), e = dot(b0, o), f = dot(d1, o);
  const double den = a * c - b * b;
  const double s0 = den > 1e-12 ? (c * e - b * f) / den : 1.0, s1 = den > 1e-12 ? (b * e - a * f) / den : 1.0;
  const V3 p0 = 0.5 * (s0 * b0 + o + s1 * d1);
  const V3 pb = mul(R_b0, p0) + t_b0;
  const V3 pw = mul(R_wb, pb) + p_wb;
  pwo[3 * i] = pw.x, pwo[3 * i + 1] = pw.y, pwo[3 * i + 2] = pw.z;
}

__global__ void k_reset_state(DevState* st, int max_iterations, double radius, int spec) {
  if (threadIdx.x != 0 || blockIdx.x != 0) return;
  st->radius = radius, st->decrease_factor = 2.0;
  st->cost = st->cand_cost = st->model_cost_change = 0.0;
  st->gmax_bits = 0ull, st->gmax_pose_bits = 0ull, st->gmax = 0.0, st->x_sqnorm = st->step_sqnorm = 0.0;
  st->g_dot_step_pose = st->d2_step2_pose = st->g_dot_step_far = st->d2_step2_far = 0.0;
  st->iteration = 0, st->done = 0, st->termination = HS_NO_CONVERGENCE, st->accepted = 0, st->step_valid = 0;
  st->invalid_streak = 0, st->num_successful = 0, st->num_iterations = 0, st->scaling_ready = 0;
  st->max_iterations = max_iterations, st->chol_failed = 0;
  st->spec = spec, st->rec_sel = 0, st->rec_pending = 0;
}

__global__ void __launch_bounds__(kBlock) k_manifold_plus(int kind, int ambient, int tangent, int n, const double* __restrict__ x,
                                                          const double* __restrict__ d, double* __restrict__ out, double* __restrict__ jac) {
  const int i = blockIdx.x * blockDim.x + threadIdx.x;
  if (i >= n) return;
  const double* xi = x + size_t(i) * ambient;
  if (out) {
    const double* di = d + size_t(i) * tangent;
    double* o = out + size_t(i) * ambient;
    switch (kind) {
      case 1:
        for (int c = 0; c < ambient; ++c) o[c] = xi[c] + di[c];
        break;
      case 2:
      case 3: {
        const Quat q = quat_plus(Quat{xi[0], xi[1], xi[2], xi[3]}, V3{di[0], di[1], di[2]});
        o[0] = q.x, o[1] = q.y, o[2] = q.z, o[3] = q.w;
        o[4] = xi[4] + di[3], o[5] = xi[5] + di[4], o[6] = xi[6] + di[5];
        if (kind == 2) o[7] = xi[7];
        break;
      }
      case 4: sphere_plus(xi, di, o); break;
      case 5:
        o[0] = xi[0] + di[0], o[1] = xi[1] + di[1], o[2] = xi[2] + di[2], o[3] = xi[3];
        break;
      default:
        for (int c = 0; c < ambient; ++c) o[c] = xi[c];
    }
  }
  if (jac && tangent > 0) {
    double* J = jac + size_t(i) * ambient * tangent;
    for (int e = 0; e < ambient * tangent; ++e) J[e] = 0.0;
    switch (kind) {
      case 1:
        for (int c = 0; c < ambient; ++c) J[c * tangent + c] = 1.0;
        break;
      case 2:
      case 3: {
        const Quat q = Quat{xi[0], xi[1], xi[2], xi[3]};
        const Quat c0 = qmul(Quat{1, 0, 0, 0}, q), c1 = qmul(Quat{0, 1, 0, 0}, q), c2 = qmul(Quat{0, 0, 1, 0}, q);
        J[0 * 6 + 0] = c0.x, J[1 * 6 + 0] = c0.y, J[2 * 6 + 0] = c0.z, J[3 * 6 + 0] = c0.w;
        J[0 * 6 + 1] = c1.x, J[1 * 6 + 1] = c1.y, J[2 * 6 + 1] = c1.z, J[3 * 6 + 1] = c1.w;
        J[0 * 6 + 2] = c2.x, J[1 * 6 + 2] = c2.y, J[2 * 6 + 2] = c2.z, J[3 * 6 + 2] = c2.w;
        J[4 * 6 + 3] = 1.0, J[5 * 6 + 4] = 1.0, J[6 * 6 + 5] = 1.0;
        break;
      }
      case 4: sphere_plus_jacobian(xi, J); break;
      case 5: J[0 * 3 + 0] = 1.0, J[1 * 3 + 1] = 1.0, J[2 * 3 + 2] = 1.0; break;
      default: break;
    }
  }
}

__global__ void __launch_bounds__(kBlock) k_manifold_minus(int kind, int ambient, int tangent, int n, const double* __restrict__ y,
                                                           const double* __restrict__ x, double* __restrict__ out, double* __restrict__ jac) {
  const int i = blockIdx.x * blockDim.x + threadIdx.x;
  if (i >= n) return;
  const double* xi = x + size_t(i) * ambient;
  if (out) {
    const double* yi = y + size_t(i) * ambient;
    double* o = out + size_t(i) * tangent;
    switch (kind) {
      case 1:
        for (int c = 0; c < ambient; ++c) o[c] = yi[c] - xi[c];
        break;
      case 2:
      case 3: {
        const V3 d = quat_minus(Quat{yi[0], yi[1], yi[2], yi[3]}, Quat{xi[0], xi[1], xi[2], xi[3]});
        o[0] = d.x, o[1] = d.y, o[2] = d.z;
        o[3] = yi[4] - xi[4], o[4] = yi[5] - xi[5], o[5] = yi[6] - xi[6];
        break;
      }
      case 4: sphere_minus(yi, xi, o); break;
      case 5: o[0] = yi[0] - xi[0], o[1] = yi[1] - xi[1], o[2] = yi[2] - xi[2]; break;
      default: break;
    }
  }
  if (jac) {
    double* J = jac + size_t(i) * ambient * tangent;
    for (int e = 0; e < ambient * tangent; ++e) J[e] = 0.0;
    switch (kind) {
      case 1:
// ... 20 lines not shown
```

hyperslam_amd/csrc/kernels_build.hpp:

```cpp
#pragma once
#include "kernels_common.hpp"

namespace hs {

template <int K>
constexpr int build_rec_stride() { return compact_record<K>() + 2; }

__host__ __device__ inline int band_tile_count(int bw, int k) { return k * bw - k * (k - 1) / 2; }
HSD int band_tile_index(int rb, int d, int bw) { return d * bw - d * (d - 1) / 2 + rb; }
struct BuildStreams {
  int ns[hsd::kMaxOrder], off[hsd::kMaxOrder + 1];
};
__host__ __device__ inline BuildStreams build_streams(int bw, int k) {
  BuildStreams b;
  for (int d = 0; d < hsd::kMaxOrder; ++d) b.ns[d] = d < k ? 1 : 0;
  int used = band_tile_count(bw, k);
  bool stuck[hsd::kMaxOrder] = {false, false, false, false, false, false, false, false};
  for (;;) {
    int best = -1;
    for (int d = 0; d < k; ++d)
      if (!stuck[d] && (best < 0 || (k - d) * b.ns[best] > (k - best) * b.ns[d])) best = d;
    if (best < 0) break;
    const bool fits = used + (bw - best) * b.ns[best] <= kBlock && 2 * b.ns[best] <= 8 && (best == 0 || 2 * b.ns[best] <= b.ns[best - 1]);
    if (!fits) {
// ... 44 lines not shown
}

struct TileOps {
  double2 r, A0, A1, A2, a00, a01, a10, a11, b00, b01, b10, b11;
};
HSD TileOps tile_ops_load(const double* rec, int a, int b) {
  TileOps x;
  const double2* p = reinterpret_cast<const double2*>(rec);
  x.r = p[0], x.A0 = p[1], x.A1 = p[2], x.A2 = p[3];
  const double2* pa = reinterpret_cast<const double2*>(rec + 8 + 8 * a);
  const double2* pb = reinterpret_cast<const double2*>(rec + 8 + 8 * b);
  x.a00 = pa[0], x.a01 = pa[1], x.a10 = pa[2], x.a11 = pa[3];
  x.b00 = pb[0], x.b01 = pb[1], x.b10 = pb[2], x.b11 = pb[3];
  return x;
}
HSD void tile_ops_apply(const TileOps& x, bool diag, double* pacc, double* pg) {
  const double A[6] = {x.A0.x, x.A0.y, x.A1.x, x.A1.y, x.A2.x, x.A2.y};
  double ja[2][6], jb[2][6];
  ja[0][0] = x.a00.x, ja[0][1] = x.a00.y, ja[0][2] = x.a01.x, ja[1][0] = x.a10.x, ja[1][1] = x.a10.y, ja[1][2] = x.a11.x;
  jb[0][0] = x.b00.x, jb[0][1] = x.b00.y, jb[0][2] = x.b01.x, jb[1][0] = x.b10.x, jb[1][1] = x.b10.y, jb[1][2] = x.b11.x;
  const double na = -x.a01.y, nb = -x.b01.y;
#pragma unroll
  for (int i = 0; i < 2; ++i)
#pragma unroll
    for (int c = 0; c < 3; ++c) ja[i][3 + c] = na * A[3 * i + c], jb[i][3 + c] = nb * A[3 * i + c];
#pragma unroll
  for (int r = 0; r < 6; ++r)
#pragma unroll
    for (int c = 0; c < 6; ++c) pacc[6 * r + c] = fma(ja[0][r], jb[0][c], fma(ja[1][r], jb[1][c], pacc[6 * r + c]));
  if (diag) {
#pragma unroll
    for (int r = 0; r < 6; ++r) pg[r] = fma(ja[0][r], x.r.x, fma(ja[1][r], x.r.y, pg[r]));
  }
}
struct WOps {
  double2 A0, A1, A2, j00, j01, j10, j11;
};
HSD WOps w_ops_load(const double* rec, int jj) {
  WOps x;
  const double2* p = reinterpret_cast<const double2*>(rec);
  x.A0 = p[1], x.A1 = p[2], x.A2 = p[3];
  const double2* pj = reinterpret_cast<const double2*>(rec + 8 + 8 * jj);
  x.j00 = pj[0], x.j01 = pj[1], x.j10 = pj[2], x.j11 = pj[3];
  return x;
}
HSD void w_ops_apply(const WOps& x, double* wacc) {
  const double A[6] = {x.A0.x, x.A0.y, x.A1.x, x.A1.y, x.A2.x, x.A2.y};
  double jp[2][6];
  jp[0][0] = x.j00.x, jp[0][1] = x.j00.y, jp[0][2] = x.j01.x, jp[1][0] = x.j10.x, jp[1][1] = x.j10.y, jp[1][2] = x.j11.x;
  const double nb = -x.j01.y;
#pragma unroll
  for (int i = 0; i < 2; ++i)
#pragma unroll
    for (int c = 0; c < 3; ++c) jp[i][3 + c] = nb * A[3 * i + c];
#pragma unroll
  for (int r = 0; r < 6; ++r)
#pragma unroll
    for (int c = 0; c < 3; ++c) wacc[3 * r + c] = fma(jp[0][r], A[c], fma(jp[1][r], A[3 + c], wacc[3 * r + c]));
}

constexpr int kFoldFlag = 3;
HSD void pack_decision_body(const Tables& T, int decide_here, double* red, unsigned* publish);
HSD unsigned fold_wait(const Tables& T, unsigned* slot) {
  if (threadIdx.x == 0) {
    const long long t0 = wall_clock64();
    unsigned f;
    while (((f = __hip_atomic_load(T.join_flag + kFoldFlag, __ATOMIC_RELAXED, __HIP_MEMORY_SCOPE_AGENT)) >> 2) < T.fold_epoch) {
      __builtin_amdgcn_s_sleep(2);
      if (wall_clock64() - t0 > 200000000ll) {
        give_up(T.st);
        f = (T.fold_epoch << 2) | 2u;
        break;
      }
    }
    *slot = f;
  }
  __syncthreads();
  return *slot;
}

template <int K>
__global__ void __launch_bounds__(kBlock, 2) k_build_visual(Tables T, int R, int Lmax, int robustify) {
  HS_DYNAMIC_LDS(smem);
  const int fold = T.fold_decision;
  const int w = int(blockIdx.x) - fold, tid = threadIdx.x, lane = tid & 63, wave = tid >> 6;
  DevState* st = T.st;
  if (w < 0) {
    pack_decision_body(T, 3, smem, T.join_flag + kFoldFlag);
    return;
  }
  const int4 d0 = *reinterpret_cast<const int4*>(T.ch_desc + 8 * w);
  const int4 d1 = *reinterpret_cast<const int4*>(T.ch_desc + 8 * w + 4);
  const int nres = d1.x;
  const int chunk_id = d1.y;
  int st_done = 0, st_spec = 0, st_accepted = 0, st_ready = 0;
  double radius = 0.0;
  if (!fold) {
    st_done = st->done, st_spec = st->spec, st_accepted = st->accepted, st_ready = st->scaling_ready;
    radius = st->radius;
    if (st_done) return;
    if (w >= T.n_chunk) {
      if (tid == 0) T.cost_part[w] = 0.0, T.ch_gmax[w] = 0.0;
      return;
    }
  }
  constexpr int CS = build_rec_stride<K>();
  const int bw = T.bw, R6 = 6 * bw, ntile = bw * (bw + 1) / 2, nband = band_tile_count(bw, K), nseg = bw - K + 1;
  const unsigned bw_magic = ((1u << 20) + bw - 1) / bw;
  const BuildLds lay = build_lds_layout(K, bw, R, Lmax);
  double* recs = smem + lay.rec;
  double* Wy = smem + lay.wy;
  double* hbr = Wy;
  double* cps_l = smem + lay.cps;
  RelPre* relp = reinterpret_cast<RelPre*>(smem + lay.relp);
  double* lmp = smem + lay.lmp;
  double* cams = smem + lay.cam;
  double* Hb = smem + lay.hb;
  double* Linv = smem + lay.linv;
  double* cpart = smem + lay.cpart;
  int* lp = reinterpret_cast<int*>(smem + lay.ints);
  int* l_ncp = lp + Lmax + 1;
  int* l_yoff = l_ncp + Lmax;
  int* seg_start = l_yoff + Lmax;
  int* wave_cnt = seg_start + bw + 2;
  int* slot_lm = wave_cnt + 4 * bw;
  int* pos = slot_lm + R;
  uint8_t* frozen = reinterpret_cast<uint8_t*>(pos + nseg * (Lmax + 1));
  int* lane_tile = pos + nseg * (Lmax + 1) + (bw + 3) / 4;

  const bool bprof = prof_enabled(T.debug_flags, 32) && lane == 0 && w < 1023;
  long long* blog = reinterpret_cast<long long*>(T.xpart) + 48 * 1024 + 64 * w + 16 * wave;
#define HS_BSTAMP(i) \
  if (bprof) blog[i] = wall_clock64()
  HS_BSTAMP(0);

  const int lo = d0.x, nl = d0.y, cf = d0.z, q0 = d0.w;
  const int rt = R > 128 ? tid : wave == 0 ? lane : wave == 2 ? 64 + lane : kBlock;
  const bool has_rec = rt < nres;
  int my_o = -1, my_l = 0;
  VisualIn in;
  int camid = 0;
  if (has_rec) {
    const int q = q0 + rt;
    in.first = T.v_first[q], my_l = T.v_lm[q] - lo;
    my_o = in.first - cf;
    const int info = T.v_info[q];
    in.type = info >> 16, camid = info & 0xffff;
    in.stamp = T.v_stamp[q];
    in.meas[0] = T.v_meas[3 * q], in.meas[1] = T.v_meas[3 * q + 1], in.meas[2] = T.v_meas[3 * q + 2];
  }
  double f_c0x = 0.0, f_c0y = 0.0, f_c1x = 0.0, f_c1y = 0.0;
  double f_l0x = 0.0, f_l0y = 0.0, f_l0z = 0.0, f_l1x = 0.0, f_l1y = 0.0, f_l1z = 0.0;
  const int ncp_w = min(bw, T.sp.n_cp - cf);
  if (fold) {
    st_spec = st->spec;
    if (w >= T.n_chunk) {
      if (tid == 0) T.cost_part[w] = 0.0, T.ch_gmax[w] = 0.0;
      return;
    }
    st_ready = 1;
    if (tid < 4 * ncp_w) {
      const double2 c0 = reinterpret_cast<const double2*>(T.cp + 8 * cf)[tid], c1 = reinterpret_cast<const double2*>(T.cp_cand + 8 * cf)[tid];
      f_c0x = c0.x, f_c0y = c0.y, f_c1x = c1.x, f_c1y = c1.y;
    }
    if (tid < nl) {
      const double *l0 = T.lm + 3 * (lo + tid), *l1 = T.lm_cand + 3 * (lo + tid);
      f_l0x = l0[0], f_l0y = l0[1], f_l0z = l0[2], f_l1x = l1[0], f_l1y = l1[1], f_l1z = l1[2];
    }
  }
  const bool fresh = !st_ready;
  {
    if (tid < ncp_w) frozen[tid] = T.cp_const[cf + tid];
    for (int e = tid; e < 16 * min(T.n_cam, kBuildCams); e += kBlock) cams[e] = T.cam[e];
    if (tid <= nl) lp[tid] = T.lm_ptr[lo + tid] - q0;
    if (tid < nl) {
      const int dl = lo + tid;
      l_ncp[tid] = T.lm_ncp[dl], l_yoff[tid] = T.lm_yoff[dl];
      double* li = Linv + kLinv * tid;
      li[6] = fresh ? 1.0 : T.lm_scale[3 * dl], li[7] = fresh ? 1.0 : T.lm_scale[3 * dl + 1], li[8] = fresh ? 1.0 : T.lm_scale[3 * dl + 2];
      li[9] = T.lm_const[dl] ? 0.0 : 1.0;
    }
    if (!fold) {
      const bool pend = st_spec == 4 && st_accepted;
      const double* lm_src = pend ? T.lm_cand : T.lm;
      const double2* s2 = reinterpret_cast<const double2*>(T.cp + 8 * cf);
      for (int e = tid; e < 4 * ncp_w; e += kBlock) reinterpret_cast<double2*>(cps_l)[e] = s2[e];
      if (tid < nl) lmp[4 * tid] = lm_src[3 * (lo + tid)], lmp[4 * tid + 1] = lm_src[3 * (lo + tid) + 1], lmp[4 * tid + 2] = lm_src[3 * (lo + tid) + 2];
    }
  }
  int my_rank = 0;
  for (int o = 0; o < nseg; ++o) {
    const unsigned long long m = __ballot(my_o == o);
    if (my_o == o) my_rank = __popcll(m & ((1ull << lane) - 1ull));
    if (lane == 0) wave_cnt[wave * bw + o] = __popcll(m);
  }
  __syncthreads();
  HS_BSTAMP(1);
  if (wave == 1 && !fold) {
    if (lane + 1 < ncp_w) relp[lane] = rel_precompute(cps_l + 8 * lane, cps_l + 8 * lane + 8);
  }
  if (wave == 0) {
    const int tot = lane < nseg ? wave_cnt[lane] + wave_cnt[bw + lane] + wave_cnt[2 * bw + lane] + wave_cnt[3 * bw + lane] : 0;
    int inc = tot;
#pragma unroll
    for (int d = 1; d < 64; d <<= 1) {
      const int up = __shfl_up(inc, d);
      if (lane >= d) inc += up;
    }
    if (lane < nseg) seg_start[lane + 1] = inc;
    if (lane == 0) seg_start[0] = 0;
  }
  __syncthreads();
  int my_slot = 0;
  if (has_rec) {
    my_slot = seg_start[my_o] + my_rank;
    for (int ww = 0; ww < wave; ++ww) my_slot += wave_cnt[ww * bw + my_o];
    slot_lm[my_slot] = my_l;
  }
  for (int e = tid; e < nseg * (Lmax + 1); e += kBlock) pos[e] = seg_start[e / (Lmax + 1) + 1];
  if (fold) {
    const unsigned f = fold_wait(T, reinterpret_cast<unsigned*>(cpart));
    radius = __hip_atomic_load(&st->radius, __ATOMIC_RELAXED, __HIP_MEMORY_SCOPE_AGENT);
    if ((f >> 1) & 1) return;
    const bool acc = f & 1;
    if (tid < 4 * ncp_w) reinterpret_cast<double2*>(cps_l)[tid] = make_double2(acc ? f_c1x : f_c0x, acc ? f_c1y : f_c0y);
    if (tid < nl) lmp[4 * tid] = acc ? f_l1x : f_l0x, lmp[4 * tid + 1] = acc ? f_l1y : f_l0y, lmp[4 * tid + 2] = acc ? f_l1z : f_l0z;
    __syncthreads();
    if (wave == 1 && lane + 1 < ncp_w) relp[lane] = rel_precompute(cps_l + 8 * lane, cps_l + 8 * lane + 8);
  }
  __syncthreads();
  HS_BSTAMP(2);
  const bool dyn = nband <= 64 && !(HS_PROFILE_HOOKS && T.debug_flags < 0);
  if (dyn && wave == 3) {
    int t_rb = lane, t_d = 0;
#pragma unroll
    for (int d = 0; d + 1 < K; ++d)
      if (t_d == d && t_rb >= bw - d) t_rb -= bw - d, t_d = d + 1;
    const bool t_ok = lane < nband;
    int cnt = 0;
    if (t_ok) {
      const int o_hi = min(t_rb, nseg - 1), o_lo = max(0, t_rb + t_d - K + 1);
      if (o_hi >= o_lo) cnt = seg_start[o_hi + 1] - seg_start[o_lo];
    }
    constexpr int kCand[14] = {2, 3, 4, 5, 6, 7, 8, 10, 12, 16, 24, 32, 64, 256};
    int lg_sel = 0;
    bool found = false;
#pragma unroll
    for (int c = 0; c < 14; ++c) {
      const int q = (cnt + kCand[c] - 1) / kCand[c];
      const int lg = (q > 1) + (q > 2) + (q > 4) + (q > 8);
      const int lanes = __popcll(__ballot(t_ok && lg == 0)) + 2 * __popcll(__ballot(t_ok && lg == 1)) + 4 * __popcll(__ballot(t_ok && lg == 2)) +
                        8 * __popcll(__ballot(t_ok && lg == 3)) + 16 * __popcll(__ballot(t_ok && lg == 4));
      if (!found && lanes <= kBlock) found = true, lg_sel = lg;
    }
    int base = 0, my_off = 0;
#pragma unroll
    for (int c = 4; c >= 0; --c) {
      const unsigned long long m = __ballot(t_ok && lg_sel == c);
      if (t_ok && lg_sel == c) my_off = base + (__popcll(m & ((1ull << lane) - 1ull)) << c);
      base += __popcll(m) << c;
    }
#pragma unroll
    for (int j = 0; j < kBlock / 64; ++j) lane_tile[64 * j + lane] = -1;
    wait_lds();
    if (t_ok)
      for (int e = 0; e < (1 << lg_sel); ++e) lane_tile[my_off + e] = t_rb | (t_d << 8) | (lg_sel << 12);
  }
  if (has_rec) {
    const int l_prev = my_slot > seg_start[my_o] ? slot_lm[my_slot - 1] : -1;
    for (int l = l_prev + 1; l <= my_l; ++l) pos[my_o * (Lmax + 1) + l] = my_slot;
    double* rec = recs + my_slot * CS;
    in.cam = camid < kBuildCams ? cams + 16 * camid : T.cam + kCamStride * camid;
    in.lm[0] = lmp[4 * my_l], in.lm[1] = lmp[4 * my_l + 1], in.lm[2] = lmp[4 * my_l + 2];
    const double cost = visual_linearize_compact<K>(T, cps_l - 8 * cf, relp - cf, frozen - cf, in, robustify != 0, rec);
    const double a0 = rec[2], a1 = rec[3], a2 = rec[4], a3 = rec[5], a4 = rec[6], a5 = rec[7], r0 = rec[0], r1 = rec[1];
    double* h = hbr + 10 * rt;
    h[0] = fma(a0, a0, a3 * a3), h[1] = fma(a0, a1, a3 * a4), h[2] = fma(a0, a2, a3 * a5);
    h[3] = fma(a1, a1, a4 * a4), h[4] = fma(a1, a2, a4 * a5), h[5] = fma(a2, a2, a5 * a5);
    h[6] = fma(a0, r0, a3 * r1), h[7] = fma(a1, r0, a4 * r1), h[8] = fma(a2, r0, a5 * r1);
    h[9] = cost;
  }
  HS_BSTAMP(3);
  __syncthreads();
  HS_BSTAMP(4);
  if (tid < 9 * nl) {
    const int l = tid / 9, e = tid - 9 * l;
    double acc = 0.0;
    for (int t = lp[l]; t < lp[l + 1]; ++t) acc += hbr[10 * t + e];
    Hb[10 * l + e] = acc;
  } else if (tid >= kBlock - 8) {
    const int g = tid - (kBlock - 8), per = (nres + 7) / 8;
    double acc = 0.0;
    for (int t = g * per; t < min(nres, (g + 1) * per); ++t) acc += hbr[10 * t + 9];
    cpart[g] = acc;
  }
  __syncthreads();
  const int n_task_w = nl * bw;
  for (int tau = tid; tau < n_task_w; tau += kBlock) {
    const int l = int((unsigned(tau) * bw_magic) >> 20), jb = tau - l * bw;
    double wacc[18];
#pragma unroll
    for (int e = 0; e < 18; ++e) wacc[e] = 0.0;
    int run_lo[K], cum[K];
    int total = 0;
    const bool in_rows = jb < l_ncp[l];
#pragma unroll
    for (int jj = 0; jj < K; ++jj) {
      const int o = jb - jj;
      const bool ok = in_rows && o >= 0 && o < nseg;
      const int* pp = pos + (ok ? o : 0) * (Lmax + 1) + l;
      const int a = pp[0], b = pp[1];
      run_lo[jj] = a, total += ok ? b - a : 0, cum[jj] = total;
    }
#define HS_W_LOAD(h_, dst)                                                   \
  {                                                                          \
    int jj_ = 0, s_ = run_lo[0] + (h_);                                      \
    _Pragma("unroll") for (int x = 1; x < K; ++x) if ((h_) >= cum[x - 1]) jj_ = x, s_ = run_lo[x] + (h_)-cum[x - 1]; \
    dst = w_ops_load(recs + s_ * CS, jj_);                                   \
  }
    WOps opa, opb;
    if (total > 0) HS_W_LOAD(0, opa);
    for (int h = 0; h < total; h += 2) {
      if (h + 1 < total) HS_W_LOAD(h + 1, opb);
      w_ops_apply(opa, wacc);
      if (h + 1 < total) {
        if (h + 2 < total) HS_W_LOAD(h + 2, opa);
        w_ops_apply(opb, wacc);
      }
    }
#undef HS_W_LOAD
    double* wr = Wy + (size_t(l) * R6 + 6 * jb) * 3;
#pragma unroll
    for (int e = 0; e < 18; e += 2) *reinterpret_cast<double2*>(wr + e) = make_double2(wacc[e], wacc[e + 1]);
  }
  HS_BSTAMP(5);
  int p_d = 0, p_off = 0, ns_lg = 0, p_end = 0;
#pragma unroll
  for (int d = 0; d < K; ++d) {
    const int lg = (T.build_stream_lg >> (2 * d)) & 3, next = p_end + ((bw - d) << lg);
    if (tid >= p_end && tid < next) p_d = d, p_off = p_end, ns_lg = lg;
    p_end = next;
  }
  bool p_lane = tid < p_end;
  int p_rb = p_lane ? (tid - p_off) >> ns_lg : 0;
  if (dyn) {
    const int lt = lane_tile[tid];
    p_lane = lt >= 0;
    p_rb = p_lane ? lt & 255 : 0, p_d = p_lane ? (lt >> 8) & 15 : 0, ns_lg = p_lane ? (lt >> 12) & 7 : 0, p_off = 0;
  }
  const int NS = 1 << ns_lg, ns0 = 1 << (T.build_stream_lg & 3);
  const int p_s = (tid - p_off) & (NS - 1);
  const bool lv2 = dyn ? __ballot(ns_lg > 1) != 0 : ns0 > 2, lv4 = dyn ? __ballot(ns_lg > 2) != 0 : ns0 > 4, lv8 = dyn && __ballot(ns_lg > 3) != 0;
  const int p_tb = band_tile_index(p_rb, p_d, bw);
// ... 522 lines not shown
```

hyperslam_amd/csrc/kernels_common.hpp:

```cpp
#pragma once
#include <type_traits>
#include "factors.hpp"
#include "device_primitives.hpp"

namespace hs {

constexpr int kBlock = 256;

#ifndef HS_PROFILE_HOOKS
#define HS_PROFILE_HOOKS 0
#endif
constexpr int kDenseLd = 256;
HSD bool prof_enabled(int debug_flags, int bit) { return HS_PROFILE_HOOKS && (debug_flags & bit); }

constexpr int kGatherFlag = 4 + 2 * 512 + 512 + 4 * kProgressStride;

HSD void give_up(DevState* st) {
  st->chol_failed = 2;
  st->termination = HS_FAILURE;
  st->done = 1;
}


template <int CTRL>
HSD double dpp_move(double v) {
  const int lo = __builtin_amdgcn_update_dpp(0, __double2loint(v), CTRL, 0xF, 0xF, false);
  const int hi = __builtin_amdgcn_update_dpp(0, __double2hiint(v), CTRL, 0xF, 0xF, false);
  return __hiloint2double(hi, lo);
}
HSD double lane_xor1(double v) { return dpp_move<0xB1>(v); }
HSD double lane_xor2(double v) { return dpp_move<0x4E>(v); }
HSD double lane_xor4(double v) {
  const double up = dpp_move<0x104>(v), down = dpp_move<0x114>(v);
  return (threadIdx.x & 4) ? down : up;
}

HSD double wave_sum(double v) {
  v += __shfl_xor(v, 32);
  v += __shfl_xor(v, 16);
  v += dpp_move<0x128>(v);
  v += lane_xor4(v);
  v += lane_xor2(v);
  v += lane_xor1(v);
  return v;
}
HSD double wave_sum_fast(double v) { return wave_sum(v); }


HSD double block_sum(double v, double* lds ) {
  v = wave_sum(v);
  const int w = threadIdx.x >> 6;
  if ((threadIdx.x & 63) == 0) lds[w] = v;
  __syncthreads();
  double s = 0;
  if (threadIdx.x == 0)
    for (int i = 0; i < int(blockDim.x >> 6); ++i) s += lds[i];
  __syncthreads();
  return s;
}

template <int N>
HSD void block_sum_n(double (&v)[N], double* lds ) {
  const int w = threadIdx.x >> 6, nw = int(blockDim.x >> 6);
#pragma unroll
  for (int e = 0; e < N; ++e) {
    v[e] = wave_sum_fast(v[e]);
    if ((threadIdx.x & 63) == 0) lds[e * nw + w] = v[e];
  }
  __syncthreads();
  if (threadIdx.x == 0) {
#pragma unroll
    for (int e = 0; e < N; ++e) {
      double s = 0;
      for (int i = 0; i < nw; ++i) s += lds[e * nw + i];
      v[e] = s;
    }
  }
  __syncthreads();
}

HSD double strided_sum(const double* __restrict__ p, int n, int stride = 1, int offset = 0) {
  double s = 0.0;
  for (int i0 = threadIdx.x; i0 < n; i0 += 8 * blockDim.x) {
    double v[8];
#pragma unroll
    for (int u = 0; u < 8; ++u) {
      const int i = i0 + u * blockDim.x;
      v[u] = i < n ? p[size_t(i) * stride + offset] : 0.0;
    }
#pragma unroll
    for (int u = 0; u < 8; ++u) s += v[u];
  }
  return s;
}
template <int U = 8>
HSD double strided_max(const double* __restrict__ p, int n) {
  double m = 0.0;
  for (int i0 = threadIdx.x; i0 < n; i0 += U * blockDim.x) {
    double v[U];
#pragma unroll
    for (int u = 0; u < U; ++u) {
      const int i = i0 + u * blockDim.x;
      v[u] = i < n ? p[i] : 0.0;
// ... 35 lines not shown
```

hyperslam_amd/csrc/kernels_update.hpp:

```cpp
#pragma once
#include "kernels_common.hpp"

namespace hs {

template <bool CALIB = false>
__global__ void __launch_bounds__(kBlock) k_backsub_retract(Tables T) {
  if (T.st->done) return;
  __shared__ double red[kBlock / 64][4];
  const bool pend = T.st->spec == 2 && T.st->accepted;
  if (int(blockIdx.x) < T.n_lm_part) {
    const int lane = threadIdx.x & 63, wave = threadIdx.x >> 6;
    const int dl = blockIdx.x * (kBlock / 64) + wave;
    double xl = 0.0, sl = 0.0, gd = 0.0, dd = 0.0;
    if (dl < T.n_lm) {
      const int rows = 6 * T.lm_ncp[dl], r0 = 6 * T.lm_cfirst[dl];
      const double* Y = T.Y + T.lm_yoff[dl];
      double L[6] = {1, 0, 1, 0, 0, 1}, yh[3] = {0, 0, 0}, x[3] = {0, 0, 0}, sc[3] = {0, 0, 0}, sb[3] = {0, 0, 0}, d2[3] = {0, 0, 0};
      bool active = false;
      if (lane == 0) {
#pragma unroll
        for (int a = 0; a < 6; ++a) L[a] = T.lm_L[6 * dl + a];
#pragma unroll
        for (int a = 0; a < 3; ++a) {
          yh[a] = T.lm_yhat[3 * dl + a], x[a] = (pend ? T.lm_cand : T.lm)[3 * dl + a], sc[a] = T.lm_scale[3 * dl + a];
// ... 112 lines not shown
  if (st->done) return;
  double gm = strided_max(T.gabs, T.np + T.nb);
#pragma unroll
  for (int o = 32; o > 0; o >>= 1) gm = fmax(gm, __shfl_xor(gm, o));
  if ((threadIdx.x & 63) == 0) red[threadIdx.x >> 6] = gm;
  __syncthreads();
  if (threadIdx.x != 0) return;
  for (int i = 1; i < int(blockDim.x >> 6); ++i) gm = fmax(gm, red[i]);
  const double c = T.xbuf[T.xo_cost];
  for (int r = 0; r < T.world; ++r) gm = fmax(gm, T.xbuf[T.xo_gmax + r]);
  begin_iteration(T, c, gm, true);
}

HSD void begin_iteration(const Tables& T, double c, double gm, bool set_scaling_ready) {
  DevState* st = T.st;
  st->cost = c;
  st->gmax = gm;
  if (set_scaling_ready) st->scaling_ready = 1;
  if (st->iteration == 0) {
    hs_iteration& r = st->records[0];
    r.iteration = 0, r.step_is_valid = 1, r.step_is_successful = 1, r.cost = c, r.cost_change = 0, r.gradient_max_norm = gm;
    r.step_norm = 0, r.relative_decrease = 0, r.radius = st->radius;
    st->iteration = 1;
  } else {
    st->records[st->iteration - 1].gradient_max_norm = gm;
  }
  if (st->iteration - 1 >= st->max_iterations) {
    st->done = 1, st->termination = HS_NO_CONVERGENCE;
  } else if (gm <= 1e-10) {
    st->done = 1, st->termination = HS_CONVERGENCE;
  } else if (st->radius <= 1e-32) {
    st->done = 1, st->termination = HS_CONVERGENCE;
  }
}

struct DecideIn {
  double g_pose, g_far, d2_pose, d2_far, cost, gmax, radius, decrease_factor;
  int chol_failed, iteration, rec_pending, invalid_streak;
};
HSD DecideIn decide_inputs(const DevState* st) {
  DecideIn in;
  in.g_pose = st->g_dot_step_pose, in.g_far = st->g_dot_step_far, in.d2_pose = st->d2_step2_pose, in.d2_far = st->d2_step2_far;
  in.cost = st->cost, in.gmax = st->gmax, in.radius = st->radius, in.decrease_factor = st->decrease_factor;
  in.chol_failed = st->chol_failed, in.iteration = st->iteration, in.rec_pending = st->rec_pending, in.invalid_streak = st->invalid_streak;
  return in;
}

HSD void decide_step(const Tables& T, const double* D_known, const DecideIn& in);
HSD void decide_step(const Tables& T, const double* D_known = nullptr);
HSD void commit_body(const Tables& T, int idx, int stride);
HSD void commit_control_points(const Tables& T, int idx, int stride);

HSD void pack_decision_body(const Tables& T, const int decide_here, double* red , unsigned* publish) {
  DevState* st = T.st;
  const int done_at_entry = st->done;
  const bool dprof = prof_enabled(T.debug_flags, 32) && publish && threadIdx.x == 0;
  long long* dlog = reinterpret_cast<long long*>(T.xpart) + 48 * 1024 + 64 * 1023;
  if (dprof) dlog[0] = wall_clock64();
  DecideIn din = {};
  if (threadIdx.x == 0 && decide_here) din = decide_inputs(st);
  double cand = 0.0, xs = 0.0, ss = 0.0, gd = 0.0, dd = 0.0;
  const int n_max = max(T.n_cost_part, max(T.n_lm_part, T.n_norm_part));
  const bool with_replicated = T.rank == 0;
  for (int i0 = threadIdx.x; i0 < n_max; i0 += 4 * kBlock) {
    double c[4];
    double2 la[4], lb[4], nr[4];
#pragma unroll
    for (int u = 0; u < 4; ++u) {
      const int i = i0 + u * kBlock;
      c[u] = i < T.n_cost_part ? T.cand_part[i] : 0.0;
      const double2* lp = reinterpret_cast<const double2*>(T.lm_part) + 2 * size_t(i);
      la[u] = i < T.n_lm_part ? lp[0] : make_double2(0.0, 0.0);
      lb[u] = i < T.n_lm_part ? lp[1] : make_double2(0.0, 0.0);
      nr[u] = (with_replicated && i < T.n_norm_part) ? reinterpret_cast<const double2*>(T.norm_part)[i] : make_double2(0.0, 0.0);
    }
#pragma unroll
    for (int u = 0; u < 4; ++u) {
      cand += c[u];
      xs += la[u].x, ss += la[u].y, gd += lb[u].x, dd += lb[u].y;
      xs += nr[u].x, ss += nr[u].y;
    }
  }
  if (done_at_entry) {
    if (publish && threadIdx.x == 0) __hip_atomic_store(publish, (T.fold_epoch << 2) | 2u, __ATOMIC_RELEASE, __HIP_MEMORY_SCOPE_AGENT);
    return;
  }
  double v5[5] = {cand, xs, ss, gd, dd};
  if (dprof) dlog[1] = wall_clock64();
  block_sum_n<5>(v5, red);
  if (dprof) dlog[2] = wall_clock64();
  int* accepted = reinterpret_cast<int*>(red + 5 * (kBlock / 64));
  if (threadIdx.x == 0) {
    double* D = T.xbuf + T.xo_dec;
#pragma unroll
    for (int e = 0; e < 5; ++e) D[e] = v5[e];
    st->local_cand = v5[0];
    if (decide_here) decide_step(T, v5, din);
    if (decide_here >= 2) *accepted = st->accepted;
    if (dprof) dlog[3] = wall_clock64();
    if (publish)
      __hip_atomic_store(publish, (T.fold_epoch << 2) | (st->done ? 2u : 0u) | (st->accepted ? 1u : 0u), __ATOMIC_RELEASE, __HIP_MEMORY_SCOPE_AGENT);
    if (dprof) dlog[4] = wall_clock64();
  }
  if (decide_here >= 2) {
    __syncthreads();
    if (*accepted && decide_here == 2) commit_body(T, threadIdx.x, blockDim.x);
    if (*accepted && decide_here == 3) commit_control_points(T, threadIdx.x, blockDim.x);
  }
}

__global__ void __launch_bounds__(kBlock) k_pack_decision(Tables T, int decide_here ) {
  __shared__ double red[5 * (kBlock / 64) + 1];
  pack_decision_body(T, decide_here, red, nullptr);
}

HSD void decide_step(const Tables& T, const double* D_known, const DecideIn& in) {
  DevState* st = T.st;
  const double* D = D_known ? D_known : T.xbuf + T.xo_dec;
  const double cand = D[0], xs = D[1], ss = D[2];
  const double g_step = (in.g_pose + in.g_far) + D[3], d_step = (in.d2_pose + in.d2_far) + D[4];
  const double mcc = -0.5 * g_step + 0.5 * d_step;
  st->model_cost_change = mcc;
  st->scaling_ready = 1;
  const int step_valid = (isfinite(mcc) && !in.chol_failed && mcc > 0.0) ? 1 : 0;
  st->step_valid = step_valid;
  const int it = in.iteration;
  hs_iteration& r = st->records[it];
  r.iteration = it, r.cost = in.cost, r.cost_change = 0, r.gradient_max_norm = in.gmax, r.step_norm = 0, r.relative_decrease = 0;
  r.step_is_valid = step_valid, r.step_is_successful = 0;
  st->num_iterations = it;
  st->accepted = 0;
  const int rec_pending = in.rec_pending;
  st->rec_pending = 0;
  st->gmax_bits = 0ull, st->gmax_pose_bits = 0ull;
  double radius = in.radius;
  if (!step_valid) {
    if (in.invalid_streak + 1 >= 5) {
      st->done = 1, st->termination = HS_FAILURE;
    } else {
      radius *= 0.5;
      st->radius = radius;
      if (in.chol_failed == 1) st->chol_failed = 0;
    }
    st->invalid_streak = in.invalid_streak + 1;
    r.radius = radius;
    st->iteration = it + 1;
    return;
  }
  st->invalid_streak = 0;
  st->cand_cost = cand;
  const double step_norm = sqrt(ss);
  r.step_norm = step_norm;
  if (step_norm <= 1e-8 * (sqrt(xs) + 1e-8)) {
    st->done = 1, st->termination = HS_CONVERGENCE;
    r.radius = radius;
    return;
  }
  const double cost_change = in.cost - cand;
  r.cost_change = cost_change;
  if (fabs(cost_change) <= 1e-6 * in.cost) {
    st->done = 1, st->termination = HS_CONVERGENCE;
    r.radius = radius;
    return;
  }
  const double relative_decrease = (in.cost - cand) / mcc;
  r.relative_decrease = relative_decrease;
  if (relative_decrease > 1e-3) {
    r.step_is_successful = 1;
    st->accepted = 1;
    st->num_successful++;
    st->cost = cand;
    st->local_cost = st->local_cand;
    if (rec_pending) st->rec_sel ^= 1;
    r.cost = cand;
    const double q = 2.0 * relative_decrease - 1.0;
    radius = fmin(1e16, radius / fmax(1.0 / 3.0, 1.0 - q * q * q));
    st->decrease_factor = 2.0;
  } else {
    r.cost = cand;
    radius = radius / in.decrease_factor;
    st->decrease_factor = in.decrease_factor * 2.0;
  }
  st->radius = radius;
  r.radius = radius;
  st->iteration = it + 1;
}
HSD void decide_step(const Tables& T, const double* D_known) { decide_step(T, D_known, decide_inputs(T.st)); }

__global__ void __launch_bounds__(kBlock) k_decide(Tables T, int commit_cps) {
  if (T.st->done) return;
  __shared__ int accepted;
  if (threadIdx.x == 0) {
    decide_step(T);
    accepted = T.st->accepted;
  }
  __syncthreads();
  if (commit_cps && accepted) commit_control_points(T, threadIdx.x, blockDim.x);
}

HSD void commit_body(const Tables& T, const int idx, const int stride) {
  auto copy = [&](double* __restrict__ dst, const double* __restrict__ src, int n) {
    for (int e0 = idx; e0 < n; e0 += 8 * stride) {
      double v[8];
#pragma unroll
      for (int u = 0; u < 8; ++u) {
        const int e = e0 + u * stride;
        v[u] = e < n ? src[e] : 0.0;
      }
#pragma unroll
      for (int u = 0; u < 8; ++u) {
        const int e = e0 + u * stride;
        if (e < n) dst[e] = v[u];
      }
    }
  };
  copy(T.cp, T.cp_cand, 8 * T.sp.n_cp);
  copy(T.lm, T.lm_cand, 3 * T.n_lm);
  if (T.nb > T.nc) {
    for (int e = idx; e < 4 * T.n_bias; e += stride) T.bias_g[e] = T.bias_g_cand[e], T.bias_a[e] = T.bias_a_cand[e];
    if (idx < 3) T.gravity[idx] = T.gravity_cand[idx];
  }
}

HSD void commit_control_points(const Tables& T, const int idx, const int stride) {
  for (int e0 = idx; e0 < 8 * T.sp.n_cp; e0 += 4 * stride) {
    double v[4];
#pragma unroll
    for (int u = 0; u < 4; ++u) v[u] = e0 + u * stride < 8 * T.sp.n_cp ? T.cp_cand[e0 + u * stride] : 0.0;
#pragma unroll
    for (int u = 0; u < 4; ++u)
      if (e0 + u * stride < 8 * T.sp.n_cp) T.cp[e0 + u * stride] = v[u];
  }
}

constexpr int kCommitInline = 4096;

__global__ void __launch_bounds__(kBlock) k_commit(Tables T) {
  if (T.st->accepted) commit_body(T, blockIdx.x * blockDim.x + threadIdx.x, gridDim.x * blockDim.x);
}

}
```

hyperslam_amd/csrc/problem.hpp:

```cpp
#pragma once
#include <hip/hip_runtime.h>
#include <stdint.h>

#include "../../include/hyperslam_hip.h"
#include "device_math.hpp"

namespace hs {

constexpr int kMaxIterations = 64;
constexpr int kCamStride = 16;

struct Spline {
  int k, n_cp;
  double t0, dt, inv_dt;
  int rot_const, trans_const;
};

struct DevState {
  double radius, decrease_factor;
  double cost;
  double cand_cost;
  double local_cost;
  double local_cand;
  double model_cost_change;
  unsigned long long gmax_bits;
  unsigned long long gmax_pose_bits;
  double gmax;
  double x_sqnorm, step_sqnorm;
  double g_dot_step_pose, d2_step2_pose;
  double g_dot_step_far, d2_step2_far;
  int iteration;
  int done;
  int termination;
  int accepted;
  int step_valid;
  int invalid_streak;
  int num_successful;
  int num_iterations;
  int scaling_ready;
  int max_iterations;
  int chol_failed;
  int spec;
  int rec_sel;
  int rec_pending;
  hs_iteration records[kMaxIterations + 1];
};

struct FactorJob {
  const double* Sb;
  const double* g_s;
  double* Ub;
  double* Ubk;
  double* ybuf;
  double* win;
  int n_steps;
  int merge_at;
};

constexpr int kProgressStride = 32;

struct MfmaJob {
  const double* L;
  const double* g;
  double* Ub;
  double* Ubk;
  double* ybuf;
  double* win;
  int n_steps;
  int merge_at;
  int enter_limit;
  int zero_from;
  int dump;
  const double* zero;
  unsigned* progress;
  unsigned progress_base;
};

struct Tables {
  Spline sp;
  hsd::BasisCoef basis;
  double* cp;
  double* cp_cand;
  const uint8_t* cp_const;
  const double* cam;
  int n_cam;
  const double* sensor;
  int n_lm;
  double* lm;
  double* lm_cand;
  const uint8_t* lm_const;
  const int* lm_ptr;
  const int* lm_cfirst;
  const int* lm_ncp;
  const int* lm_yoff;
  const int* cf_ptr;
  double* lm_scale;
  double* lm_L;
  double* lm_yhat;
  double* lm_sb;
  double* lm_D2;
  double* lm_part;
  int n_lm_part;
  double* lm_gmax;
  int n_obs_lm;
  double* Y;
  int n_vis;
  const double* v_stamp;
  const double* v_meas;
  const int* v_lm;
  const int* v_info;
  const int* v_first;
  const int* v_pos;
  double* v_rec;
  double* v_rec_alt;
  const int* v_seg_ptr;
  int n_pri;
  const double* p_stamp;
  const double* p_meas;
  const int* p_sensor;
  const int* p_first;
  double* p_rec;
  const int* p_seg_ptr;
  int n_seg;
  int n_ine;
  const double* i_stamp;
  const double* i_meas;
  const int* i_first;
  const int* i_first_bias;
  double* i_rec;
  const int* i_seg_ptr;
  const struct ImuParams* imu;
  hsd::BasisCoef bias_basis;
  int kb, n_bias;
  double bias_t0, bias_dt;
  double* bias_g;
  double* bias_a;
  double* bias_g_cand;
  double* bias_a_cand;
  double* gravity;
  double* gravity_cand;
  int bias_const, gravity_const;
  int inertial_literal;
  int nb;
  int nc;
  const int* calib_map;
  double* calib_rec;
  double* calib_Yc;
  double* calib_part;
  int bw;
  int np;
  double* scale_p;
  double* Sb;
  double* Ub;
  double* Ubk;
  double* g_s;
  double* g_full;
  double* D2p;
  double* gabs;
  double* step_p;
  double* delta_p;
  double* ybuf;
  double* ybuf2;
  int y_split;
  double* scale_b;
  double* Spb;
  double* Sbb;
  double* gb_s;
  double* D2b;
  double* Zb;
  double* Cb;
  double* hb;
  double* xb;
  double* delta_b;
  const int* i_bias_ptr;
  const int* bfwd_start;
  double* cost_part;
  double* cand_part;
  int n_cost_part;
  double* norm_part;
  int n_norm_part;
  double* xbuf;
  const int* sw_ptr;
  const int* sw_seg;
  FactorJob fj[2];
  MfmaJob mj[2];
  double* Sb2;
  double* g2;
  double* xsol;
  unsigned* join_flag;
  unsigned join_epoch;
  unsigned gather_epoch;
  double* gravity_part;
  double* segP;
  const int* gw_ptr;
  const int* gw_cf;
  double* Qw;
  double* Yt;
  int yt_stride;
  int wide_q;
  double* grpQ;
  double* xpart;
  int xo_g, xo_gs, xo_dj, xo_pb, xo_bb, xo_gb, xo_cost, xo_gmax, xo_dec, x_count1;
  int xo_cdj;
  int fused, n_chunk;
  int build_stream_lg;
  double* ch_gmax;
  int bookkeep;
  int fold_decision;
  unsigned fold_epoch;
  const int* ch_ptr;
  const int* ch_desc;
  double* dense;
  int dense_f0;
  unsigned sweep_epoch;
  int dense_border;
  int rank, world;
  int debug_flags;
  DevState* st;
};

}
```

Measured before the change: 260.9 million.

## Fold state reset, tail commit and result readback into kernels with host mailbox

```diff
diff --git a/hyperslam_amd/csrc/capi.hip b/hyperslam_amd/csrc/capi.hip
--- a/hyperslam_amd/csrc/capi.hip
+++ b/hyperslam_amd/csrc/capi.hip
@@ -53,7 +53,14 @@
     }
     p->own_stream = true;
   }
-  if (hipHostMalloc(reinterpret_cast<void**>(&p->h_state), sizeof(DevState), hipHostMallocDefault) != hipSuccess) {
+  if (hipHostMalloc(reinterpret_cast<void**>(&p->h_mail), sizeof(hs_problem::Mailbox), hipHostMallocCoherent) != hipSuccess) {
+    delete p;
+    return HS_ERR_DEVICE;
+  }
+  std::memset(p->h_mail, 0, sizeof(hs_problem::Mailbox));
+  p->h_state = &p->h_mail->st;
+  if (hipHostGetDevicePointer(reinterpret_cast<void**>(&p->d_mail), p->h_mail, 0) != hipSuccess) {
+    (void)hipHostFree(p->h_mail);
     delete p;
     return HS_ERR_DEVICE;
   }
@@ -91,7 +98,7 @@
   if (p->ev_join) (void)hipEventDestroy(p->ev_join);
   if (p->ev_irec) (void)hipEventDestroy(p->ev_irec);
   if (p->side) (void)hipStreamDestroy(p->side);
-  if (p->h_state) (void)hipHostFree(p->h_state);
+  if (p->h_mail) (void)hipHostFree(p->h_mail);
   if (p->h_result) (void)hipHostFree(p->h_result);
   if (p->rccl_comm && rccl_api()) (void)rccl_api()->CommDestroy(static_cast<ncclComm_t>(p->rccl_comm));
   if (p->own_stream) (void)hipStreamDestroy(p->stream);
@@ -873,6 +880,12 @@
   return HS_OK;
 }
 
+static inline void cpu_pause() {
+#if defined(__x86_64__) && !defined(__HIP_DEVICE_COMPILE__)
+  __builtin_ia32_pause();
+#endif
+}
+
 int hs_solve(hs_problem* p, int max_iterations, hs_summary* summary, hs_iteration* iterations) {
   if (!p || !summary) return HS_ERR_INVALID;
   if (p->has_weights()) HS_FAIL(HS_ERR_INVALID, kWeightsMessage);
@@ -890,11 +903,18 @@
   const bool spec = speculative_solve(p);
   const bool deferred = (fused_visual_only(p) || (spec && !commit_inline(p))) && !(p->T.debug_flags & 67108864);
   const bool fold = fold_decision_into_build(p, deferred);
-  rc = reset_state(p, max_iterations, 1e4, spec ? (deferred ? 2 : 1) : (deferred ? 4 : 0));
-  if (rc) return rc;
+  const bool old_ends = (p->T.debug_flags2 & 1) != 0;
+  const bool ends_in_kernels = fold && max_iterations > 0 && !old_ends;
+  const int spec_mode = spec ? (deferred ? 2 : 1) : (deferred ? 4 : 0);
+  const FirstState first_state{max_iterations, spec_mode, 1e4};
+  if (!ends_in_kernels) {
+    rc = reset_state(p, max_iterations, 1e4, spec_mode);
+    if (rc) return rc;
+  }
   hipStream_t s = p->stream;
   const auto host_t3 = std::chrono::steady_clock::now();
   const bool stages = p->stage_timing;
+  const bool end_events = stages || old_ends;
   const size_t n_ev = size_t(6) * max_iterations + 1;
   const size_t ev_cand = size_t(4) * max_iterations + 1;
   while (p->events.size() < n_ev) {
@@ -903,7 +923,7 @@
     p->events.push_back(e);
   }
   std::vector<hipEvent_t>& ev = p->events;
-  HIP_TRY(hipEventRecord(ev[0], s));
+  if (end_events) HIP_TRY(hipEventRecord(ev[0], s));
   for (int it = 0; it < max_iterations; ++it) {
     if (it == 0 || !spec) {
       HS_ORDER_SWITCH(p->k, rc = launch_linearize<K>(p, true));
@@ -911,7 +931,7 @@
     }
     if (stages && !p->fused) HIP_TRY(hipEventRecord(ev[4 * it + 1], s));
     hipEvent_t after_build = stages && p->fused ? ev[4 * it + 1] : nullptr;
-    HS_ORDER_SWITCH(p->k, rc = launch_build<K>(p, after_build, it > 0, it > 0 && fold));
+    HS_ORDER_SWITCH(p->k, rc = launch_build<K>(p, after_build, it > 0, it > 0 && fold, it == 0 && ends_in_kernels ? &first_state : nullptr));
     if (rc) return rc;
     if (stages) HIP_TRY(hipEventRecord(ev[4 * it + 2], s));
     rc = launch_factor(p);
@@ -919,10 +939,19 @@
     if (stages) HIP_TRY(hipEventRecord(ev[4 * it + 3], s));
     const bool lin_cand = spec && it + 1 < max_iterations;
     hipEvent_t* lin_ev = stages && lin_cand ? &ev[ev_cand + 2 * it] : nullptr;
-    HS_ORDER_SWITCH(p->k, rc = launch_update<K>(p, lin_cand, deferred, lin_ev, fold && it + 1 < max_iterations));
+    const bool last = it + 1 == max_iterations;
+    HS_ORDER_SWITCH(p->k, rc = launch_update<K>(p, lin_cand, deferred, lin_ev, fold && (!last || ends_in_kernels)));
     if (rc) return rc;
-    if (deferred && it + 1 == max_iterations) launch_commit(p);
-    if (stages || it + 1 == max_iterations) HIP_TRY(hipEventRecord(ev[4 * it + 4], s));
+    if (last && ends_in_kernels) {
+      rc = launch_tail(p);
+      if (rc) return rc;
+    } else if (deferred && last)
+      launch_commit(p);
+    if (last && !ends_in_kernels && !end_events) {
+      k_stamp_end<<<1, 64, 0, s>>>(p->d_state.p);
+      HIP_TRY(hipGetLastError());
+    }
+    if (stages || (last && end_events)) HIP_TRY(hipEventRecord(ev[4 * it + 4], s));
   }
   if (max_iterations == 0) {
     HS_ORDER_SWITCH(p->k, rc = launch_linearize<K>(p, false, true));
@@ -952,8 +981,22 @@
     if (p->has_imu) HIP_TRY(hipMemcpyAsync(h + n_cp8 + n_lm3 + 2 * n_b, p->d_gravity.p, 24, hipMemcpyDeviceToHost, s));
   }
   if (p->T.nc && max_iterations > 0) HIP_TRY(hipMemcpyAsync(p->cam.data(), p->d_cam.p, p->cam.size() * 8, hipMemcpyDeviceToHost, s));
-  HIP_TRY(hipMemcpyAsync(&st, p->d_state.p, sizeof(st), hipMemcpyDeviceToHost, s));
-  HIP_TRY(hipStreamSynchronize(s));
+  if (!ends_in_kernels) HIP_TRY(hipMemcpyAsync(&st, p->d_state.p, sizeof(st), hipMemcpyDeviceToHost, s));
+  bool arrived = false;
+  if (ends_in_kernels && !end_events && !p->want_results && !(p->T.debug_flags2 & 4)) {
+    constexpr double kMailboxSpinUs = 4000.0;
+    const unsigned want = p->mail_epoch;
+    for (int spins = 0; !arrived; ++spins) {
+      arrived = __atomic_load_n(&p->h_mail->epoch, __ATOMIC_ACQUIRE) == want;
+      if (arrived) break;
+      cpu_pause();
+      if ((spins & 255) == 255 && std::chrono::duration<double, std::micro>(std::chrono::steady_clock::now() - host_t4).count() > kMailboxSpinUs) break;
+    }
+  }
+  if (!arrived) {
+    HIP_TRY(hipStreamSynchronize(s));
+    if (ends_in_kernels && __atomic_load_n(&p->h_mail->epoch, __ATOMIC_ACQUIRE) != p->mail_epoch) HS_FAIL(HS_ERR_DEVICE, "hs_solve: the solver state did not arrive");
+  }
   if (max_iterations > 0) p->device_ahead = true;
   p->results_cached = p->want_results;
   if (p->host_timing) {
@@ -974,18 +1017,20 @@
   if (!stages) summary->linearize_ms = summary->schur_ms = summary->solve_ms = summary->update_ms = -1.0;
   for (int it = 0; stages && it < max_iterations; ++it) {
     float t[4] = {0, 0, 0, 0};
-    for (int k = 0; k < 4; ++k) (void)hipEventElapsedTime(&t[k], ev[4 * it + k], ev[4 * it + k + 1]);
+    for (int k = 0; k < 4; ++k) HIP_TRY(hipEventElapsedTime(&t[k], ev[4 * it + k], ev[4 * it + k + 1]));
     summary->linearize_ms += t[0], summary->schur_ms += t[1], summary->solve_ms += t[2], summary->update_ms += t[3];
     if (spec && it + 1 < max_iterations) {
       float tc = 0;
-      (void)hipEventElapsedTime(&tc, ev[ev_cand + 2 * it], ev[ev_cand + 2 * it + 1]);
+      HIP_TRY(hipEventElapsedTime(&tc, ev[ev_cand + 2 * it], ev[ev_cand + 2 * it + 1]));
       summary->linearize_ms += tc, summary->update_ms -= tc;
     }
   }
-  if (max_iterations > 0) {
+  if (max_iterations > 0 && end_events) {
     float t = 0;
-    (void)hipEventElapsedTime(&t, ev[0], ev[4 * max_iterations]);
+    HIP_TRY(hipEventElapsedTime(&t, ev[0], ev[4 * max_iterations]));
     summary->total_ms = t;
+  } else if (max_iterations > 0) {
+    summary->total_ms = double(st.t_end - st.t_begin) * 1e-5;
   }
   if (iterations) {
     std::memset(iterations, 0, sizeof(hs_iteration) * (size_t(max_iterations) + 1));
@@ -1032,12 +1077,32 @@
   if (!p->has_snapshot || p->dirty) HS_FAIL(HS_ERR_STATE, "hs_restore without a valid hs_snapshot");
   p->results_cached = false;
   p->cov_valid = false;
-  HIP_TRY(hipMemcpyAsync(p->d_cp.p, p->d_cp_snap.p, p->cp.size() * 8, hipMemcpyDeviceToDevice, p->stream));
-  if (p->n_lm) HIP_TRY(hipMemcpyAsync(p->d_lm.p, p->d_lm_snap.p, p->lm.size() * 8, hipMemcpyDeviceToDevice, p->stream));
-  if (p->has_imu) {
-    HIP_TRY(hipMemcpyAsync(p->d_bias_g.p, p->d_bias_g_snap.p, p->bias_g.size() * 8, hipMemcpyDeviceToDevice, p->stream));
-    HIP_TRY(hipMemcpyAsync(p->d_bias_a.p, p->d_bias_a_snap.p, p->bias_a.size() * 8, hipMemcpyDeviceToDevice, p->stream));
-    HIP_TRY(hipMemcpyAsync(p->d_gravity.p, p->d_gravity_snap.p, 24, hipMemcpyDeviceToDevice, p->stream));
+  if (p->T.debug_flags2 & 1) {
+    HIP_TRY(hipMemcpyAsync(p->d_cp.p, p->d_cp_snap.p, p->cp.size() * 8, hipMemcpyDeviceToDevice, p->stream));
+    if (p->n_lm) HIP_TRY(hipMemcpyAsync(p->d_lm.p, p->d_lm_snap.p, p->lm.size() * 8, hipMemcpyDeviceToDevice, p->stream));
+    if (p->has_imu) {
+      HIP_TRY(hipMemcpyAsync(p->d_bias_g.p, p->d_bias_g_snap.p, p->bias_g.size() * 8, hipMemcpyDeviceToDevice, p->stream));
+      HIP_TRY(hipMemcpyAsync(p->d_bias_a.p, p->d_bias_a_snap.p, p->bias_a.size() * 8, hipMemcpyDeviceToDevice, p->stream));
+      HIP_TRY(hipMemcpyAsync(p->d_gravity.p, p->d_gravity_snap.p, 24, hipMemcpyDeviceToDevice, p->stream));
+    }
+  } else {
+    RestoreJobs J = {};
+    size_t total = 0;
+    int a = 0;
+    auto add = [&](double* dst, const double* src, size_t n) {
+      if (n) J.dst[a] = dst, J.src[a] = src, J.n[a] = int(n), ++a, total += n;
+    };
+    add(p->d_cp.p, p->d_cp_snap.p, p->cp.size());
+    if (p->n_lm) add(p->d_lm.p, p->d_lm_snap.p, p->lm.size());
+    if (p->has_imu) {
+      add(p->d_bias_g.p, p->d_bias_g_snap.p, p->bias_g.size());
+      add(p->d_bias_a.p, p->d_bias_a_snap.p, p->bias_a.size());
+      add(p->d_gravity.p, p->d_gravity_snap.p, 3);
+    }
+    if (total) {
+      k_restore<<<int(std::min<size_t>((total + 4 * kBlock - 1) / (4 * kBlock), 1024)), kBlock, 0, p->stream>>>(J);
+      HIP_TRY(hipGetLastError());
+    }
   }
   if (p->cam != p->cam_snap && p->cam.size() == p->cam_snap.size()) {
     p->cam = p->cam_snap;
diff --git a/hyperslam_amd/csrc/host_launch.hpp b/hyperslam_amd/csrc/host_launch.hpp
--- a/hyperslam_amd/csrc/host_launch.hpp
+++ b/hyperslam_amd/csrc/host_launch.hpp
@@ -121,8 +121,12 @@
   return !factor_two_ended_any(p) && !HS_AB(T.debug_flags, 131072) && dense_mx_fits(n_blk - *f0, T.nb) && !(T.debug_flags & 8);
 }
 
+struct FirstState {
+  int max_iterations, spec;
+  double radius;
+};
 template <int K>
-int launch_build(hs_problem* p, hipEvent_t after_build = nullptr, bool scaling_fixed = false, bool fold = false) {
+int launch_build(hs_problem* p, hipEvent_t after_build = nullptr, bool scaling_fixed = false, bool fold = false, const FirstState* first_state = nullptr) {
   const Tables& T = p->T;
   hipStream_t s = p->stream;
   p->bookkeep = false;
@@ -133,6 +137,10 @@
   if (fused && fold) {
     Tables Tf = T;
     Tf.fold_decision = 1, Tf.fold_epoch = ++p->join_epoch;
+    k_build_visual<K><<<p->nb_vis + 1, kBlock, p->build_lds, s>>>(Tf, p->build_R, p->build_L, 1);
+  } else if (fused && first_state) {
+    Tables Tf = T;
+    Tf.fold_decision = 2, Tf.reset_max_iterations = first_state->max_iterations, Tf.reset_spec = first_state->spec, Tf.reset_radius = first_state->radius;
     k_build_visual<K><<<p->nb_vis + 1, kBlock, p->build_lds, s>>>(Tf, p->build_R, p->build_L, 1);
   } else if (fused)
     k_build_visual<K><<<p->nb_vis, kBlock, p->build_lds, s>>>(T, p->build_R, p->build_L, 1);
@@ -579,6 +587,19 @@
   k_commit<<<nb_commit, kBlock, 0, p->stream>>>(T);
 }
 
+static int launch_tail(hs_problem* p) {
+  const Tables& T = p->T;
+  const int nb_copy = std::max((3 * T.n_lm + kBlock - 1) / kBlock, 1);
+  Tables Tt = T;
+  Tt.fold_decision = 1, Tt.fold_epoch = ++p->join_epoch;
+  Tt.tail_target = unsigned(nb_copy);
+  Tt.mailbox_epoch = p->mail_epoch + 1;
+  k_commit<<<1 + nb_copy, kBlock, 0, p->stream>>>(Tt, 1);
+  HIP_TRY(hipGetLastError());
+  ++p->mail_epoch;
+  return HS_OK;
+}
+
 template <int K>
 static void warm_kernels_of_order() {
   hipFuncAttributes fa;
@@ -612,7 +633,8 @@
       reinterpret_cast<const void*>(&k_border_solve_reg<5>), reinterpret_cast<const void*>(&k_border_solve_reg<6>), reinterpret_cast<const void*>(&k_border_solve_reg<7>),
       reinterpret_cast<const void*>(&k_border_solve_reg<8>), reinterpret_cast<const void*>(&k_border_apply), reinterpret_cast<const void*>(&k_backsub_retract<false>),
       reinterpret_cast<const void*>(&k_pack_decision), reinterpret_cast<const void*>(&k_decide), reinterpret_cast<const void*>(&k_commit),
-      reinterpret_cast<const void*>(&k_reset_state), reinterpret_cast<const void*>(&k_scatter_uploads)};
+      reinterpret_cast<const void*>(&k_reset_state), reinterpret_cast<const void*>(&k_stamp_end), reinterpret_cast<const void*>(&k_restore),
+      reinterpret_cast<const void*>(&k_scatter_uploads)};
   for (const void* k : kernels) (void)hipFuncGetAttributes(&fa, k);
   warm_kernels_of_order<4>();
   warm_kernels_of_order<5>();
diff --git a/hyperslam_amd/csrc/host_structure.hpp b/hyperslam_amd/csrc/host_structure.hpp
--- a/hyperslam_amd/csrc/host_structure.hpp
+++ b/hyperslam_amd/csrc/host_structure.hpp
@@ -213,6 +213,73 @@
   return true;
 }
 
+constexpr int kChunkLanes = 256;
+inline int chunk_sort_stride(int k, int bw, int R, int Lmax) { return R + (bw + 2) + (bw - k + 1) * (Lmax + 1) + kChunkLanes; }
+inline void chunk_sort_tables(const int* o, const int* l, int nres, int k, int bw, int R, int Lmax, int* out) {
+  const int nseg = bw - k + 1, nband = k * bw - k * (k - 1) / 2;
+  int* slot = out;
+  int* seg_start = slot + R;
+  int* pos = seg_start + bw + 2;
+  int* lane_tile = pos + nseg * (Lmax + 1);
+  for (int e = 0; e < chunk_sort_stride(k, bw, R, Lmax); ++e) out[e] = 0;
+  for (int t = 0; t < nres; ++t)
+    if (o[t] >= 0 && o[t] < nseg) seg_start[o[t] + 1]++;
+  for (int s = 0; s < nseg; ++s) seg_start[s + 1] += seg_start[s];
+  {
+    std::vector<int> cur(seg_start, seg_start + nseg);
+    for (int t = 0; t < nres; ++t)
+      if (o[t] >= 0 && o[t] < nseg) slot[t] = cur[o[t]]++;
+  }
+  for (int s = 0; s < nseg; ++s)
+    for (int x = 0; x <= Lmax; ++x) pos[s * (Lmax + 1) + x] = seg_start[s + 1];
+  for (int t = nres - 1; t >= 0; --t)
+    if (o[t] >= 0 && o[t] < nseg)
+      for (int x = std::min(l[t], Lmax); x >= 0 && pos[o[t] * (Lmax + 1) + x] > slot[t]; --x) pos[o[t] * (Lmax + 1) + x] = slot[t];
+  for (int e = 0; e < kChunkLanes; ++e) lane_tile[e] = -1;
+  if (nband > 64) return;
+  int t_rb[64], t_d[64], cnt[64], lg_sel[64];
+  for (int i = 0; i < nband; ++i) {
+    int rb = i, d = 0;
+    while (d + 1 < k && rb >= bw - d) rb -= bw - d, ++d;
+    t_rb[i] = rb, t_d[i] = d;
+    const int o_hi = std::min(rb, nseg - 1), o_lo = std::max(0, rb + d - k + 1);
+    cnt[i] = o_hi >= o_lo ? seg_start[o_hi + 1] - seg_start[o_lo] : 0;
+  }
+  const int cand[14] = {2, 3, 4, 5, 6, 7, 8, 10, 12, 16, 24, 32, 64, 256};
+  for (int c = 0; c < 14; ++c) {
+    int lanes = 0;
+    for (int i = 0; i < nband; ++i) {
+      const int q = (cnt[i] + cand[c] - 1) / cand[c];
+      lg_sel[i] = (q > 1) + (q > 2) + (q > 4) + (q > 8);
+      lanes += 1 << lg_sel[i];
+    }
+    if (lanes <= kChunkLanes) break;
+  }
+  int base = 0;
+  for (int c = 4; c >= 0; --c)
+    for (int i = 0; i < nband; ++i)
+      if (lg_sel[i] == c) {
+        for (int e = 0; e < (1 << c); ++e) lane_tile[base + e] = t_rb[i] | (t_d[i] << 8) | (c << 12);
+        base += 1 << c;
+      }
+}
+
+inline void build_chunk_sort_tables(const VisualStructure& vs, int k, int R, int Lmax, const std::vector<int>& ch_desc, std::vector<int>* out) {
+  const int n = int(ch_desc.size() / 8), stride = chunk_sort_stride(k, vs.bw, R, Lmax);
+  out->assign(size_t(n) * stride + 1, 0);
+  std::vector<int> o, l;
+  for (int w = 0; w < n; ++w) {
+    const int* d = ch_desc.data() + 8 * w;
+    const int lo = d[0], cf = d[2], q0 = d[3], nres = d[4];
+    o.resize(nres), l.resize(nres);
+    for (int t = 0, dl = lo; t < nres; ++t) {
+      while (vs.lm_ptr[dl + 1] <= q0 + t) ++dl;
+      o[t] = vs.first[q0 + t] - cf, l[t] = dl - lo;
+    }
+    chunk_sort_tables(o.data(), l.data(), nres, k, vs.bw, R, Lmax, out->data() + size_t(w) * stride);
+  }
+}
+
 inline void order_chunks_for_dispatch(const VisualStructure& vs, int k, int n_cu, std::vector<int>* ch_desc, int n) {
   if (n <= 1 || n_cu <= 0) return;
   std::vector<int> weight(n), order(n);
diff --git a/hyperslam_amd/csrc/host_tables.hpp b/hyperslam_amd/csrc/host_tables.hpp
--- a/hyperslam_amd/csrc/host_tables.hpp
+++ b/hyperslam_amd/csrc/host_tables.hpp
@@ -282,9 +282,9 @@
   bool bookkeep = false;
   int build_R = 0, build_L = 0;
   size_t build_lds = 0;
-  DBuf<int> d_ch_ptr, d_ch_desc;
+  DBuf<int> d_ch_ptr, d_ch_desc, d_ch_sort;
   DBuf<double> d_ch_gmax;
-  std::vector<int> h_ch_ptr, h_gw_ptr, h_gw_cf, h_ch_desc;
+  std::vector<int> h_ch_ptr, h_gw_ptr, h_gw_cf, h_ch_desc, h_ch_sort;
   DBuf<double> d_ybuf, d_scale_b, d_Spb, d_Sbb, d_gb_s, d_D2b, d_Zb, d_Cb, d_hb, d_xb, d_delta_b, d_bias_g_snap, d_bias_a_snap, d_gravity_snap;
   DBuf<int> d_i_bias_ptr, d_bfwd_start;
   int n_split = 1;
@@ -292,6 +292,13 @@
   DBuf<double> d_cp_snap, d_lm_snap;
   bool has_snapshot = false;
   DevState* h_state = nullptr;
+  struct Mailbox {
+    DevState st;
+    unsigned epoch;
+  };
+  Mailbox* h_mail = nullptr;
+  unsigned long long* d_mail = nullptr;
+  unsigned mail_epoch = 0;
   bool cov_valid = false;
   int cov_np = 0, cov_ncb = 0, cov_nb = 0, cov_nlm = 0;
   DBuf<double> d_cov_U, d_cov_sig, d_cov_Z, d_cov_X, d_cov_C, d_cov_Li, d_cov_band, d_cov_pb, d_cov_bb, d_cov_lm;
@@ -753,6 +760,9 @@
       HIP_TRY(p->d_gw_cf.upload(p->h_gw_cf, s));
       HIP_TRY(p->d_ch_ptr.upload(p->h_ch_ptr, s));
       HIP_TRY(p->d_ch_desc.upload(p->h_ch_desc, s));
+      static_assert(kChunkLanes == kBlock, "lane_tile has one entry per lane of k_build_visual");
+      build_chunk_sort_tables(vs, k, p->build_R, p->build_L, p->h_ch_desc, &p->h_ch_sort);
+      HIP_TRY(p->d_ch_sort.upload(p->h_ch_sort, s));
       p->n_group_wg = int(p->h_ch_ptr.size()) - 1;
     } else {
       for (int c = 0; c < p->n_cp; ++c) {
@@ -823,6 +833,9 @@
   T.fj[1] = FactorJob{nullptr, nullptr, nullptr, nullptr, nullptr, nullptr, 0, -1};
   T.xsol = p->d_xsol.p, T.join_flag = p->d_join.p, T.join_epoch = 0;
   T.debug_flags = std::getenv("HS_DEBUG_FLAGS") ? std::atoi(std::getenv("HS_DEBUG_FLAGS")) : 0;
+  T.debug_flags2 = std::getenv("HS_DEBUG_FLAGS2") ? std::atoi(std::getenv("HS_DEBUG_FLAGS2")) : 0;
+  T.reset_max_iterations = 0, T.reset_spec = 0, T.reset_radius = 0.0;
+  T.tail_ticket = p->d_join.p + kTailTicket, T.tail_target = 0, T.mailbox = p->d_mail, T.mailbox_epoch = 0;
   {
     const bool la_ok = la_compute_waves(vs.bw) > 0, two_ended = la_ok && np / 6 >= 4 * vs.bw;
     const bool need = two_ended || (HS_AB(T.debug_flags, 131072) && mfma_window_tiles(vs.bw) > 0);
@@ -832,6 +845,8 @@
   T.Zb = p->d_Zb.p, T.Cb = p->d_Cb.p, T.hb = p->d_hb.p, T.xb = p->d_xb.p, T.delta_b = p->d_delta_b.p, T.i_bias_ptr = p->d_i_bias_ptr.p, T.bfwd_start = p->nc ? p->d_calib_bfwd.p : p->d_bfwd_start.p;
   T.x_count1 = x_count1, T.xo_dec = x_count1, T.xo_cdj = x_count0;
   T.fused = p->fused ? 1 : 0, T.n_chunk = p->fused ? p->n_group_wg : 0, T.ch_ptr = p->d_ch_ptr.p, T.ch_desc = p->d_ch_desc.p;
+  const bool staged_sort = p->fused && !(std::getenv("HS_DEBUG_FLAGS2") && (std::atoi(std::getenv("HS_DEBUG_FLAGS2")) & 2));
+  T.ch_sort = staged_sort ? p->d_ch_sort.p : nullptr, T.ch_sort_stride = p->fused ? chunk_sort_stride(k, vs.bw, p->build_R, p->build_L) : 0;
   T.build_stream_lg = p->fused ? build_streams_packed(vs.bw, k) : 0;
   T.ch_gmax = p->d_ch_gmax.p;
   T.rank = p->rank, T.world = p->world;
diff --git a/hyperslam_amd/csrc/kernels_aux.hpp b/hyperslam_amd/csrc/kernels_aux.hpp
--- a/hyperslam_amd/csrc/kernels_aux.hpp
+++ b/hyperslam_amd/csrc/kernels_aux.hpp
@@ -72,14 +72,34 @@
 
 __global__ void k_reset_state(DevState* st, int max_iterations, double radius, int spec) {
   if (threadIdx.x != 0 || blockIdx.x != 0) return;
-  st->radius = radius, st->decrease_factor = 2.0;
-  st->cost = st->cand_cost = st->model_cost_change = 0.0;
-  st->gmax_bits = 0ull, st->gmax_pose_bits = 0ull, st->gmax = 0.0, st->x_sqnorm = st->step_sqnorm = 0.0;
-  st->g_dot_step_pose = st->d2_step2_pose = st->g_dot_step_far = st->d2_step2_far = 0.0;
-  st->iteration = 0, st->done = 0, st->termination = HS_NO_CONVERGENCE, st->accepted = 0, st->step_valid = 0;
-  st->invalid_streak = 0, st->num_successful = 0, st->num_iterations = 0, st->scaling_ready = 0;
-  st->max_iterations = max_iterations, st->chol_failed = 0;
-  st->spec = spec, st->rec_sel = 0, st->rec_pending = 0;
+  reset_state_body(st, max_iterations, radius, spec);
+}
+
+__global__ void k_stamp_end(DevState* st) {
+  if (threadIdx.x == 0 && blockIdx.x == 0) st->t_end = wall_clock64();
+}
+
+struct RestoreJobs {
+  double* dst[5];
+  const double* src[5];
+  int n[5];
+};
+__global__ void __launch_bounds__(kBlock) k_restore(RestoreJobs J) {
+  const int idx = blockIdx.x * blockDim.x + threadIdx.x, stride = gridDim.x * blockDim.x;
+#pragma unroll
+  for (int a = 0; a < 5; ++a) {
+    const int n = J.n[a];
+    const double* __restrict__ src = J.src[a];
+    double* __restrict__ dst = J.dst[a];
+    for (int e0 = idx; e0 < n; e0 += 4 * stride) {
+      double v[4];
+#pragma unroll
+      for (int u = 0; u < 4; ++u) v[u] = e0 + u * stride < n ? src[e0 + u * stride] : 0.0;
+#pragma unroll
+      for (int u = 0; u < 4; ++u)
+        if (e0 + u * stride < n) dst[e0 + u * stride] = v[u];
+    }
+  }
 }
 
 __global__ void __launch_bounds__(kBlock) k_manifold_plus(int kind, int ambient, int tangent, int n, const double* __restrict__ x,
diff --git a/hyperslam_amd/csrc/kernels_build.hpp b/hyperslam_amd/csrc/kernels_build.hpp
--- a/hyperslam_amd/csrc/kernels_build.hpp
+++ b/hyperslam_amd/csrc/kernels_build.hpp
@@ -150,11 +150,16 @@
 template <int K>
 __global__ void __launch_bounds__(kBlock, 2) k_build_visual(Tables T, int R, int Lmax, int robustify) {
   HS_DYNAMIC_LDS(smem);
-  const int fold = T.fold_decision;
-  const int w = int(blockIdx.x) - fold, tid = threadIdx.x, lane = tid & 63, wave = tid >> 6;
+  const int fold = T.fold_decision == 1, first = T.fold_decision == 2;
+  const int w = int(blockIdx.x) - (fold | first), tid = threadIdx.x, lane = tid & 63, wave = tid >> 6;
   DevState* st = T.st;
   if (w < 0) {
-    pack_decision_body(T, 3, smem, T.join_flag + kFoldFlag);
+    if (fold)
+      pack_decision_body(T, 3, smem, T.join_flag + kFoldFlag);
+    else if (tid == 0) {
+      reset_state_body(st, T.reset_max_iterations, T.reset_radius, T.reset_spec);
+      __hip_atomic_store(T.tail_ticket, 0u, __ATOMIC_RELAXED, __HIP_MEMORY_SCOPE_AGENT);
+    }
     return;
   }
   const int4 d0 = *reinterpret_cast<const int4*>(T.ch_desc + 8 * w);
@@ -164,8 +169,12 @@
   int st_done = 0, st_spec = 0, st_accepted = 0, st_ready = 0;
   double radius = 0.0;
   if (!fold) {
-    st_done = st->done, st_spec = st->spec, st_accepted = st->accepted, st_ready = st->scaling_ready;
-    radius = st->radius;
+    if (first)
+      st_spec = T.reset_spec, radius = T.reset_radius;
+    else {
+      st_done = st->done, st_spec = st->spec, st_accepted = st->accepted, st_ready = st->scaling_ready;
+      radius = st->radius;
+    }
     if (st_done) return;
     if (w >= T.n_chunk) {
       if (tid == 0) T.cost_part[w] = 0.0, T.ch_gmax[w] = 0.0;
@@ -256,8 +265,17 @@
       if (tid < nl) lmp[4 * tid] = lm_src[3 * (lo + tid)], lmp[4 * tid + 1] = lm_src[3 * (lo + tid) + 1], lmp[4 * tid + 2] = lm_src[3 * (lo + tid) + 2];
     }
   }
+  const int* sort_tab = T.ch_sort ? T.ch_sort + size_t(w) * T.ch_sort_stride : nullptr;
+  const bool staged = sort_tab != nullptr;
+  int my_slot = 0;
+  if (staged) {
+    if (has_rec) my_slot = sort_tab[rt];
+    for (int e = tid; e < nseg + 1; e += kBlock) seg_start[e] = sort_tab[R + e];
+    for (int e = tid; e < nseg * (Lmax + 1); e += kBlock) pos[e] = sort_tab[R + bw + 2 + e];
+    lane_tile[tid] = sort_tab[R + bw + 2 + nseg * (Lmax + 1) + tid];
+  }
   int my_rank = 0;
-  for (int o = 0; o < nseg; ++o) {
+  for (int o = 0; o < nseg && !staged; ++o) {
     const unsigned long long m = __ballot(my_o == o);
     if (my_o == o) my_rank = __popcll(m & ((1ull << lane) - 1ull));
     if (lane == 0) wave_cnt[wave * bw + o] = __popcll(m);
@@ -267,7 +285,7 @@
   if (wave == 1 && !fold) {
     if (lane + 1 < ncp_w) relp[lane] = rel_precompute(cps_l + 8 * lane, cps_l + 8 * lane + 8);
   }
-  if (wave == 0) {
+  if (wave == 0 && !staged) {
     const int tot = lane < nseg ? wave_cnt[lane] + wave_cnt[bw + lane] + wave_cnt[2 * bw + lane] + wave_cnt[3 * bw + lane] : 0;
     int inc = tot;
 #pragma unroll
@@ -278,14 +296,13 @@
     if (lane < nseg) seg_start[lane + 1] = inc;
     if (lane == 0) seg_start[0] = 0;
   }
-  __syncthreads();
-  int my_slot = 0;
-  if (has_rec) {
+  if (!staged) __syncthreads();
+  if (has_rec && !staged) {
     my_slot = seg_start[my_o] + my_rank;
     for (int ww = 0; ww < wave; ++ww) my_slot += wave_cnt[ww * bw + my_o];
     slot_lm[my_slot] = my_l;
   }
-  for (int e = tid; e < nseg * (Lmax + 1); e += kBlock) pos[e] = seg_start[e / (Lmax + 1) + 1];
+  for (int e = tid; e < nseg * (Lmax + 1) && !staged; e += kBlock) pos[e] = seg_start[e / (Lmax + 1) + 1];
   if (fold) {
     const unsigned f = fold_wait(T, reinterpret_cast<unsigned*>(cpart));
     radius = __hip_atomic_load(&st->radius, __ATOMIC_RELAXED, __HIP_MEMORY_SCOPE_AGENT);
@@ -299,7 +316,7 @@
   __syncthreads();
   HS_BSTAMP(2);
   const bool dyn = nband <= 64 && !(HS_PROFILE_HOOKS && T.debug_flags < 0);
-  if (dyn && wave == 3) {
+  if (dyn && wave == 3 && !staged) {
     int t_rb = lane, t_d = 0;
 #pragma unroll
     for (int d = 0; d + 1 < K; ++d)
@@ -335,8 +352,10 @@
       for (int e = 0; e < (1 << lg_sel); ++e) lane_tile[my_off + e] = t_rb | (t_d << 8) | (lg_sel << 12);
   }
   if (has_rec) {
-    const int l_prev = my_slot > seg_start[my_o] ? slot_lm[my_slot - 1] : -1;
-    for (int l = l_prev + 1; l <= my_l; ++l) pos[my_o * (Lmax + 1) + l] = my_slot;
+    if (!staged) {
+      const int l_prev = my_slot > seg_start[my_o] ? slot_lm[my_slot - 1] : -1;
+      for (int l = l_prev + 1; l <= my_l; ++l) pos[my_o * (Lmax + 1) + l] = my_slot;
+    }
     double* rec = recs + my_slot * CS;
     in.cam = camid < kBuildCams ? cams + 16 * camid : T.cam + kCamStride * camid;
     in.lm[0] = lmp[4 * my_l], in.lm[1] = lmp[4 * my_l + 1], in.lm[2] = lmp[4 * my_l + 2];
diff --git a/hyperslam_amd/csrc/kernels_common.hpp b/hyperslam_amd/csrc/kernels_common.hpp
--- a/hyperslam_amd/csrc/kernels_common.hpp
+++ b/hyperslam_amd/csrc/kernels_common.hpp
@@ -19,6 +19,24 @@
   st->chol_failed = 2;
   st->termination = HS_FAILURE;
   st->done = 1;
+}
+
+#ifdef HS_EMULATED_DEVICE
+#define __HIP_MEMORY_SCOPE_SYSTEM __HIP_MEMORY_SCOPE_AGENT
+inline void __threadfence_system() { __threadfence(); }
+#endif
+constexpr int kTailTicket = kGatherFlag + 3;
+
+HSD void reset_state_body(DevState* st, int max_iterations, double radius, int spec) {
+  st->radius = radius, st->decrease_factor = 2.0;
+  st->cost = st->cand_cost = st->model_cost_change = 0.0;
+  st->gmax_bits = 0ull, st->gmax_pose_bits = 0ull, st->gmax = 0.0, st->x_sqnorm = st->step_sqnorm = 0.0;
+  st->g_dot_step_pose = st->d2_step2_pose = st->g_dot_step_far = st->d2_step2_far = 0.0;
+  st->iteration = 0, st->done = 0, st->termination = HS_NO_CONVERGENCE, st->accepted = 0, st->step_valid = 0;
+  st->invalid_streak = 0, st->num_successful = 0, st->num_iterations = 0, st->scaling_ready = 0;
+  st->max_iterations = max_iterations, st->chol_failed = 0;
+  st->spec = spec, st->rec_sel = 0, st->rec_pending = 0;
+  st->t_begin = st->t_end = wall_clock64();
 }
 
 
diff --git a/hyperslam_amd/csrc/kernels_update.hpp b/hyperslam_amd/csrc/kernels_update.hpp
--- a/hyperslam_amd/csrc/kernels_update.hpp
+++ b/hyperslam_amd/csrc/kernels_update.hpp
@@ -218,7 +218,8 @@
     }
   }
   if (done_at_entry) {
-    if (publish && threadIdx.x == 0) __hip_atomic_store(publish, (T.fold_epoch << 2) | 2u, __ATOMIC_RELEASE, __HIP_MEMORY_SCOPE_AGENT);
+    if (publish && threadIdx.x == 0)
+      __hip_atomic_store(publish, (T.fold_epoch << 2) | 2u | (st->accepted ? 1u : 0u), __ATOMIC_RELEASE, __HIP_MEMORY_SCOPE_AGENT);
     return;
   }
   double v5[5] = {cand, xs, ss, gd, dd};
@@ -371,8 +372,50 @@
 
 constexpr int kCommitInline = 4096;
 
-__global__ void __launch_bounds__(kBlock) k_commit(Tables T) {
-  if (T.st->accepted) commit_body(T, blockIdx.x * blockDim.x + threadIdx.x, gridDim.x * blockDim.x);
-}
-
-}
+HSD unsigned fold_wait(const Tables& T, unsigned* slot);
+
+HSD void tail_publish(const Tables& T) {
+  DevState* st = T.st;
+  if (threadIdx.x == 0) {
+    const long long t0 = wall_clock64();
+    while (__hip_atomic_load(T.tail_ticket, __ATOMIC_RELAXED, __HIP_MEMORY_SCOPE_AGENT) < T.tail_target) {
+      __builtin_amdgcn_s_sleep(2);
+      if (wall_clock64() - t0 > 200000000ll) break;
+    }
+    st->t_end = wall_clock64();
+  }
+  __syncthreads();
+  static_assert(sizeof(DevState) % 8 == 0, "the mailbox is copied in 8-byte words");
+  const unsigned long long* src = reinterpret_cast<const unsigned long long*>(st);
+  for (int i = threadIdx.x; i < int(sizeof(DevState) / 8); i += blockDim.x)
+    __hip_atomic_store(T.mailbox + i, __hip_atomic_load(src + i, __ATOMIC_RELAXED, __HIP_MEMORY_SCOPE_AGENT), __ATOMIC_RELAXED, __HIP_MEMORY_SCOPE_SYSTEM);
+  __threadfence_system();
+  __syncthreads();
+  if (threadIdx.x == 0)
+    __hip_atomic_store(reinterpret_cast<unsigned*>(T.mailbox + sizeof(DevState) / 8), T.mailbox_epoch, __ATOMIC_RELEASE, __HIP_MEMORY_SCOPE_SYSTEM);
+}
+
+__global__ void __launch_bounds__(kBlock) k_commit(Tables T, int tail = 0) {
+  if (!tail) {
+    if (T.st->accepted) commit_body(T, blockIdx.x * blockDim.x + threadIdx.x, gridDim.x * blockDim.x);
+    return;
+  }
+  __shared__ double red[5 * (kBlock / 64) + 1];
+  __shared__ unsigned slot;
+  if (blockIdx.x == 0) {
+    pack_decision_body(T, 3, red, T.join_flag + kFoldFlag);
+    tail_publish(T);
+    return;
+  }
+  const int idx = (blockIdx.x - 1) * blockDim.x + threadIdx.x, stride = (gridDim.x - 1) * blockDim.x, n = 3 * T.n_lm;
+  const double v = idx < n ? T.lm_cand[idx] : 0.0;
+  const unsigned f = fold_wait(T, &slot);
+  if (f & 1) {
+    if (idx < n) T.lm[idx] = v;
+    for (int e = idx + stride; e < n; e += stride) T.lm[e] = T.lm_cand[e];
+  }
+  __syncthreads();
+  if (threadIdx.x == 0) atomicAdd(T.tail_ticket, 1u);
+}
+
+}
diff --git a/hyperslam_amd/csrc/problem.hpp b/hyperslam_amd/csrc/problem.hpp
--- a/hyperslam_amd/csrc/problem.hpp
+++ b/hyperslam_amd/csrc/problem.hpp
@@ -43,6 +43,7 @@
   int spec;
   int rec_sel;
   int rec_pending;
+  long long t_begin, t_end;
   hs_iteration records[kMaxIterations + 1];
 };
 
@@ -209,6 +210,8 @@
   int fold_decision;
   unsigned fold_epoch;
   const int* ch_ptr;
+  const int* ch_sort;
+  int ch_sort_stride;
   const int* ch_desc;
   double* dense;
   int dense_f0;
@@ -216,6 +219,13 @@
   int dense_border;
   int rank, world;
   int debug_flags;
+  int debug_flags2;
+  int reset_max_iterations, reset_spec;
+  double reset_radius;
+  unsigned* tail_ticket;
+  unsigned tail_target;
+  unsigned long long* mailbox;
+  unsigned mailbox_epoch;
   DevState* st;
 };
 
```

Measured after the change: 272.3 million (median of 6 runs). +4.4%, better.
